# soedinglab/spacedust

Hardware: AMD Instinct MI355X
Metric: clustersearch throughput (genome-pairs/s; SW GCUPS alongside) (higher is better)
Workload: dtype int16

## Files before the change

### include/spacedust_gpu.h

```cpp
#ifndef SPACEDUST_GPU_H
#define SPACEDUST_GPU_H

#include <stddef.h>
#include <stdint.h>

#ifdef __cplusplus
extern "C" {
#endif

enum {
    SD_OK = 0,
    SD_ENODEVICE = -1,
    SD_EHIP = -2,
    SD_EINVAL = -3,
    SD_ENOMEM = -4,
    SD_EUNSUPPORTED = -5,
    SD_EMISMATCH = -6
};

typedef struct sd_ctx sd_ctx;
typedef struct sd_seqset sd_seqset;
typedef struct sd_target sd_target;

int sd_ctx_create(int device, sd_ctx **out);
int sd_ctx_create_prio(int device, int priority, sd_ctx **out);
int sd_ctx_create_masked(int device, int priority, int reserveCUs, sd_ctx **out);
void sd_ctx_destroy(sd_ctx *ctx);
const char *sd_last_error(sd_ctx *ctx);
int sd_device_name(sd_ctx *ctx, char *buf, size_t cap);
int sd_device_memory(sd_ctx *ctx, uint64_t *freeBytes, uint64_t *totalBytes);
int sd_device_identity(int device, uint64_t *id);
int sd_workspace_report(sd_ctx *ctx, uint64_t *deviceBytes, uint64_t *pinnedBytes, char *buf, size_t cap);
int sd_workspace_release(sd_ctx *ctx);
int sd_synchronize(sd_ctx *ctx);

int sd_profile_enable(sd_ctx *ctx, int on);
int sd_profile_reset(sd_ctx *ctx);
int sd_profile_get(sd_ctx *ctx, const char *name, double *totalMs, uint64_t *launches);
int sd_profile_names(sd_ctx *ctx, char *buf, size_t cap);

int sd_seqset_create(sd_ctx *ctx, const uint8_t *residues, const uint64_t *offsets, uint32_t n,
                     const int8_t *swCompBias, sd_seqset **out);
int sd_profileset_create(sd_ctx *ctx, const uint8_t *queryLetters, const uint64_t *offsets, uint32_t n,
                         const int8_t *alnProfile, sd_seqset **out);
void sd_seqset_destroy(sd_seqset *s);

typedef struct {
    int32_t gapOpen;
    int32_t gapExtend;
    int8_t matrix[21 * 21];
    int32_t covMode;
    float covThr;
    double evalThr;
    int32_t swMode;
    uint64_t dbResidues;
} sd_sw_params;

typedef struct {
    int32_t score;
    int32_t qStart, qEnd, tStart, tEnd;
    int32_t identical;
    int32_t btLen;
    int32_t flags;
    double evalue;
    uint64_t btOffset;
} sd_sw_result;

int sd_sw_align_batch(sd_ctx *ctx, const sd_sw_params *par, const sd_seqset *queries, const sd_seqset *targets,
                      uint32_t nPairs, const uint32_t *pairQ, const uint32_t *pairT, const uint8_t *isIdentity,
                      sd_sw_result *out, char *btPool, uint64_t btCap, uint64_t *btUsed);

int sd_sw_align_batch_compact(sd_ctx *ctx, const sd_sw_params *par, const sd_seqset *queries, const sd_seqset *targets,
                              uint32_t nPairs, const uint32_t *pairQ, const uint32_t *pairT, const uint8_t *isIdentity,
                              uint32_t *outIdx, sd_sw_result *out, uint32_t *nOut, char *btPool, uint64_t btCap,
                              uint64_t *btUsed);

int sd_sw_align_batch_compact_diag(sd_ctx *ctx, const sd_sw_params *par, const sd_seqset *queries, const sd_seqset *targets,
                                   uint32_t nPairs, const uint32_t *pairQ, const uint32_t *pairT, const uint16_t *pairDiag,
                                   const uint8_t *isIdentity, uint32_t *outIdx, sd_sw_result *out, uint32_t *nOut, char *btPool,
                                   uint64_t btCap, uint64_t *btUsed);

int sd_seqset_set_groups(sd_seqset *s, const uint32_t *groupOf, uint32_t nGroups, const uint32_t *keys);
int sd_sw_align_batch_best_by_group(sd_ctx *ctx, const sd_sw_params *par, const sd_seqset *queries, const sd_seqset *targets,
                                    uint32_t nPairs, const uint32_t *pairQ, const uint32_t *pairT, const uint16_t *pairDiag,
                                    const uint8_t *isIdentity, float seqIdThr, int32_t alnLenThr, uint32_t *outIdx, sd_sw_result *out,
                                    uint32_t *nOut, char *btPool, uint64_t btCap, uint64_t *btUsed);

int sd_sw_align_alt_batch(sd_ctx *ctx, const sd_sw_params *par, const sd_seqset *queries, const sd_seqset *targets, uint32_t nSeeds,
                          const uint32_t *seedQ, const uint32_t *seedT, const int32_t *tStart, const int32_t *tEnd,
                          const uint8_t *isIdentity, uint32_t maxAlt, float seqIdThr, int32_t alnLenThr, int32_t seqIdMode,
                          sd_sw_result *out, uint32_t *outCount, char *btPool, uint64_t btCap, uint64_t *btUsed);
int sd_sw_alt_last_stats(sd_ctx *ctx, uint64_t *groups, uint64_t *seedRounds, uint64_t *bytesCopied);

int sd_sw_set_cigar_pool(sd_ctx *ctx, int on);
int sd_sw_download_bytes(sd_ctx *ctx, uint64_t *recordBytes, uint64_t *poolBytes);

int sd_sw_set_narrow_final(sd_ctx *ctx, int on);

int sd_selftest_sort_pairs(sd_ctx *ctx, const uint32_t *keys, const uint32_t *vals, uint32_t n, int beginBit, int endBit, uint32_t *outKeys,
                           uint32_t *outVals);
int sd_selftest_scan(sd_ctx *ctx, const uint32_t *in, uint32_t n, uint64_t *exclusiveSum, uint32_t *runningMax);
int sd_selftest_score_class(int kernel , int32_t n, int32_t tL, int shared, int32_t wideRowLimit,
                            uint32_t *klass, char *scope, size_t cap);
int sd_selftest_r2p_weights(sd_ctx *ctx, uint32_t nTasks, const uint32_t *nRows, const uint32_t *L, const uint8_t *cells, float *freq,
                            float *eff);

int sd_sw_align_batch_hostpath(sd_ctx *ctx, const sd_sw_params *par, const sd_seqset *queries, const sd_seqset *targets,
                               uint32_t nPairs, const uint32_t *pairQ, const uint32_t *pairT, const uint8_t *isIdentity,
                               sd_sw_result *out, char *btPool, uint64_t btCap, uint64_t *btUsed);

int sd_sw_score_batch(sd_ctx *ctx, const sd_sw_params *par, const sd_seqset *queries, const sd_seqset *targets,
                      uint32_t nPairs, const uint32_t *pairQ, const uint32_t *pairT, int lanes, int reverse,
                      const int32_t *qEnd, const int32_t *tEnd, int32_t *out);

int sd_sw_last_cells(sd_ctx *ctx, uint64_t *forwardCells, uint64_t *reverseCells, uint64_t *tracebackCells);

typedef struct {
    int32_t kmerSize;
    int32_t kmerThr;
    int32_t maxHitsPerQuery;
    int32_t minDiagScore;
    uint32_t binSize;
    int32_t covMode;
    float covThr;
    int8_t ungappedMatrix[21 * 21];
} sd_prefilter_params;

typedef struct {
    uint32_t seqId;
    int32_t score;
    uint16_t diagonal;
    uint16_t pad;
} sd_hit;

int sd_target_create(sd_ctx *ctx, int kmerSize, const uint32_t *kmerOffsets, const uint32_t *entrySeq,
                     const uint16_t *entryPos, uint64_t nEntries, const uint8_t *maskedResidues,
                     const uint64_t *seqOffsets, uint32_t nSeq, const int16_t *ext2Score, const uint16_t *ext2Index,
                     const int16_t *ext3Score, const uint16_t *ext3Index, sd_target **out);
int sd_target_create_wide(sd_ctx *ctx, int kmerSize, const uint32_t *kmerOffsets, const uint64_t *kmerBlockBase,
                          const uint32_t *entrySeq, const uint16_t *entryPos, uint64_t nEntries, const uint8_t *maskedResidues,
                          const uint64_t *seqOffsets, uint32_t nSeq, const int16_t *ext2Score, const uint16_t *ext2Index,
                          const int16_t *ext3Score, const uint16_t *ext3Index, sd_target **out);
int sd_target_build(sd_ctx *ctx, int kmerSize, int kmerThr, int mask, double maskProb, const uint8_t *residues,
                    const uint64_t *seqOffsets, uint32_t nSeq, const double *maskRatios, const int8_t *selfScore,
                    const int16_t *ext2Score, const uint16_t *ext2Index, const int16_t *ext3Score, const uint16_t *ext3Index,
                    sd_target **out, uint64_t *stats);
int sd_target_sample_check(sd_ctx *ctx, const sd_target *t, const uint32_t *kmer, const uint32_t *seq, const uint32_t *pos, uint64_t n,
                           const uint32_t *sample, uint32_t nSample, uint64_t *missing, uint64_t *inSample, uint64_t resBegin,
                           uint64_t resEnd, uint8_t *maskedOut);
int sd_target_download(sd_ctx *ctx, const sd_target *t, uint64_t *nEntries, uint64_t *tableSize, uint8_t *masked, uint64_t *starts,
                       uint32_t *entrySeq, uint16_t *entryPos);
void sd_target_destroy(sd_target *t);
uint64_t sd_target_footprint(int kmerSize, uint64_t nSeq, uint64_t nResidues);
int sd_target_build_peak(const sd_target *t, uint64_t *bytes);

int sd_prefilter_batch(sd_ctx *ctx, const sd_target *target, const sd_prefilter_params *par, uint32_t nQ,
                       const uint8_t *qResidues, const uint64_t *qOffsets, const int16_t *qKmerBias,
                       const int8_t *qDiagBias, const uint32_t *identityId, sd_hit *outHits, uint32_t *outCount,
                       uint64_t *stats);

typedef struct {
    int8_t matrix[21 * 21];
    int32_t minScore;
    int32_t maxHitsPerQuery;
    int32_t covMode;
    float covThr;
} sd_ungapped_params;
int sd_ungapped_prefilter_batch(sd_ctx *ctx, const sd_ungapped_params *par, const sd_seqset *queries, const sd_seqset *targets,
                                const uint32_t *targetKeys, const uint32_t *identityId, sd_hit *outHits, uint32_t *outCount);
int sd_ungapped_score_matrix(sd_ctx *ctx, const int8_t *matrix, const sd_seqset *queries, const sd_seqset *targets, uint8_t *out);
int sd_ungapped_last_cells(sd_ctx *ctx, uint64_t *cells);

typedef struct {
    int8_t matrix[21 * 21];
    int32_t mode;
    uint8_t aa2num[256];
} sd_rescore_params;
typedef struct {
    int32_t score;
    int32_t startPos, endPos;
// ... 285 lines not shown
```

### spacedust_amd/_lib.py

```python
import ctypes as C
import os

import numpy as np

HERE = os.path.dirname(os.path.abspath(__file__))
LIB_PATH = os.path.join(HERE, 'libsdgpu.so')

_vp = C.c_void_p


SD_OK, SD_ENODEVICE, SD_EHIP, SD_EINVAL, SD_ENOMEM, SD_EUNSUPPORTED, SD_EMISMATCH = 0, -1, -2, -3, -4, -5, -6


class SdError(RuntimeError):
    pass


class SwParams(C.Structure):
    _fields_ = [('gapOpen', C.c_int32), ('gapExtend', C.c_int32), ('matrix', C.c_int8 * 441), ('covMode', C.c_int32),
                ('covThr', C.c_float), ('evalThr', C.c_double), ('swMode', C.c_int32), ('dbResidues', C.c_uint64)]


class SwResult(C.Structure):
    _fields_ = [('score', C.c_int32), ('qStart', C.c_int32), ('qEnd', C.c_int32), ('tStart', C.c_int32),
# ... 137 lines not shown
                                            _vp, C.POINTER(_vp)]),
        'sd_host_index_block_base': (C.c_int, [_vp, C.POINTER(_vp), C.POINTER(C.c_uint64)]),
        'sd_target_destroy': (None, [_vp]),
        'sd_target_build': (C.c_int, [_vp, C.c_int, C.c_int, C.c_int, C.c_double, _vp, _vp, C.c_uint32, _vp, _vp, _vp, _vp, _vp, _vp,
                                      C.POINTER(_vp), _vp]),
        'sd_target_download': (C.c_int, [_vp, _vp, C.POINTER(C.c_uint64), C.POINTER(C.c_uint64), _vp, _vp, _vp, _vp]),
        'sd_host_index_tables': (C.c_int, [_vp, _vp, _vp]),
        'sd_target_sample_check': (C.c_int, [_vp, _vp, _vp, _vp, _vp, C.c_uint64, _vp, C.c_uint32, C.POINTER(C.c_uint64), C.POINTER(C.c_uint64),
                                             C.c_uint64, C.c_uint64, _vp]),
        'sd_device_memory': (C.c_int, [_vp, C.POINTER(C.c_uint64), C.POINTER(C.c_uint64)]),
        'sd_device_identity': (C.c_int, [C.c_int, C.POINTER(C.c_uint64)]),
        'sd_workspace_report': (C.c_int, [_vp, C.POINTER(C.c_uint64), C.POINTER(C.c_uint64), C.c_char_p, C.c_size_t]),
        'sd_workspace_release': (C.c_int, [_vp]),
        'sd_prefilter_batch': (C.c_int, [_vp, _vp, C.POINTER(PrefilterParams), C.c_uint32, _vp, _vp, _vp, _vp, _vp,
                                         _vp, _vp, _vp]),
        'sd_ungapped_prefilter_batch': (C.c_int, [_vp, C.POINTER(UngappedParams), _vp, _vp, _vp, _vp, _vp, _vp]),
        'sd_ungapped_score_matrix': (C.c_int, [_vp, _vp, _vp, _vp, _vp]),
        'sd_ungapped_last_cells': (C.c_int, [_vp, C.POINTER(C.c_uint64)]),
        'sd_seqset_set_letters': (C.c_int, [_vp, _vp]),
        'sd_rescore_diagonal_batch': (C.c_int, [_vp, C.POINTER(RescoreParams), _vp, _vp, C.c_uint32, _vp, _vp, _vp, _vp]),
        'sd_search_create_ungapped': (C.c_int, [C.c_int, C.POINTER(SearchParams), C.POINTER(SetDbView), C.POINTER(_vp)]),
        'sd_comp_bias_batch': (C.c_int, [_vp, _vp, _vp, _vp, C.c_uint32, C.c_int, _vp, _vp, _vp]),
        'sd_prefilter_profile_batch': (C.c_int, [_vp, _vp, C.POINTER(PrefilterParams), C.c_uint32, _vp, _vp, _vp, _vp, _vp,
                                                 _vp, _vp, _vp, _vp]),
        'sd_profileset_create': (C.c_int, [_vp, _vp, _vp, C.c_uint32, _vp, C.POINTER(_vp)]),
        'sd_host_map_profiles': (C.c_int, [_vp, _vp, C.c_uint32, _vp, _vp, _vp, _vp, _vp, _vp]),
        'sd_host_profile_kmer_threshold': (C.c_int, [C.c_float, C.c_int]),
        'sd_clusterhits_batch': (C.c_int, [_vp, C.POINTER(ChParams), C.c_uint32, _vp, _vp, _vp, _vp, _vp, _vp, _vp,
                                           C.c_uint32, _vp, _vp, _vp, _vp, _vp, _vp]),
        'sd_agg_create': (C.c_int, [_vp, _vp, C.c_uint32, _vp, _vp, C.c_uint32, C.c_uint32, C.c_uint32, C.c_double, C.c_int,
                                    C.c_float, C.c_int, C.c_int, C.POINTER(_vp)]),
        'sd_agg_destroy': (None, [_vp]),
        'sd_agg_add': (C.c_int, [_vp, C.c_uint32, C.c_uint32, _vp, _vp, _vp, _vp, _vp]),
        'sd_agg_finish': (C.c_int, [_vp, C.POINTER(C.c_uint64), C.POINTER(C.c_uint64)]),
        'sd_agg_stats': (C.c_int, [_vp, C.POINTER(C.c_uint64), C.POINTER(C.c_uint64)]),
        'sd_agg_get': (C.c_int, [_vp, _vp, _vp, _vp, _vp, _vp, _vp]),
        'sd_agg_write_tsv': (C.c_int, [_vp, C.c_char_p, _vp, _vp, _vp, _vp, _vp, _vp, C.c_char_p, _vp, C.c_char_p, _vp,
                                       C.c_char_p, _vp, C.c_char_p, _vp, C.c_int, C.POINTER(C.c_uint64),
                                       C.POINTER(C.c_uint64)]),
        'sd_agg_write_tsv_from': (C.c_int, [_vp, C.c_char_p, C.c_int, C.c_uint64, _vp, _vp, _vp, _vp, _vp, _vp, C.c_char_p, _vp,
                                            C.c_char_p, _vp, C.c_char_p, _vp, C.c_char_p, _vp, C.c_int, C.POINTER(C.c_uint64),
                                            C.POINTER(C.c_uint64)]),
        'sd_agg_set_keys': (C.c_int, [_vp, _vp, _vp]),
        'sd_agg_set_list_order': (C.c_int, [_vp, C.c_int]),
        'sd_agg_set_pool_form': (C.c_int, [_vp, C.c_int]),
        'sd_host_matrix_text': (C.c_int, [C.c_int, C.c_char_p, C.c_size_t]),
        'sd_host_sw_comp_bias': (C.c_int, [_vp, C.c_int, _vp, _vp, C.c_uint32, _vp]),
        'sd_host_can_be_covered': (C.c_int, [C.c_float, C.c_int, C.c_float, C.c_float]),
        'sd_host_quantise_3e': (C.c_int, [C.c_double, C.c_char_p, C.POINTER(C.c_double)]),
        'sd_host_compress_backtrace': (C.c_int, [C.c_char_p, C.c_uint64, C.c_char_p, C.c_uint64, C.POINTER(C.c_uint64)]),
        'sd_host_accept_sort': (C.c_int, [C.POINTER(AlnCriteria), C.c_uint32, C.c_uint32, _vp, _vp, _vp, _vp, _vp, _vp, _vp, _vp, _vp]),
        'sd_host_realign_select': (C.c_int, [C.POINTER(AlnCriteria), C.c_uint32, _vp, _vp, _vp, _vp, _vp, _vp, _vp, _vp, _vp, _vp,
                                             _vp, _vp]),
        'sd_alntext_create': (C.c_int, [C.POINTER(_vp)]),
        'sd_alntext_destroy': (None, [_vp]),
        'sd_alntext_format': (C.c_int, [_vp, C.POINTER(AlnCriteria), C.c_uint32, _vp, _vp, _vp, _vp, _vp, _vp, _vp, _vp, _vp]),
        'sd_alntext_get': (C.c_int, [_vp, C.POINTER(C.c_char_p), C.POINTER(_vp)]),
        'sd_search_default_params': (None, [C.POINTER(SearchParams)]),
        'sd_search_create': (C.c_int, [C.c_int, C.POINTER(SearchParams), C.POINTER(SetDbView), C.POINTER(_vp)]),
        'sd_search_create_indexed': (C.c_int, [C.c_int, C.POINTER(SearchParams), C.POINTER(SetDbView), C.POINTER(IndexView), C.POINTER(_vp)]),
        'sd_search_destroy': (None, [_vp]),
        'sd_search_last_error': (C.c_char_p, [_vp]),
        'sd_search_ctx': (_vp, [_vp, C.c_int]),
        'sd_search_target': (_vp, [_vp]),
        'sd_search_set_sinks': (C.c_int, [_vp, _vp, _vp, _vp]),
        'sd_search_set_chunk_queries': (C.c_int, [_vp, C.c_int32]),
        'sd_search_set_want_records': (C.c_int, [_vp, C.c_int]),
        'sd_search_stream': (C.c_int, [_vp, C.POINTER(SetDbView), C.c_int, C.c_uint32, _vp, _vp, _vp]),
        'sd_search_result_counts': (C.c_int, [_vp, _vp]),
        'sd_search_result_arrays': (C.c_int, [_vp] + [_vp] * 12),
        'sd_search_result_write_tsv': (C.c_int, [_vp, C.c_char_p, C.c_char_p, _vp, C.c_char_p, _vp, C.c_char_p, _vp, C.c_char_p, _vp,
                                                 C.c_int, C.c_int, C.c_uint64, C.POINTER(C.c_uint64), C.POINTER(C.c_uint64)]),
        'sd_search_result_records': (C.c_int, [_vp, _vp, C.c_uint64, C.POINTER(C.c_uint64)]),
        'sd_agg_records': (C.c_int, [_vp] * 7 + [_vp, C.c_uint64, C.POINTER(C.c_uint64)]),
        'sd_records_check': (C.c_int, [_vp, C.c_uint64, C.c_uint32, C.c_uint32, C.c_uint32, C.c_uint32, C.POINTER(C.c_uint64), C.POINTER(C.c_uint64)]),
        'sd_records_write_tsv': (C.c_int, [_vp, C.c_uint64, C.c_char_p, C.c_int, C.c_uint64, C.c_char_p, _vp, C.c_char_p, _vp, C.c_char_p, _vp,
                                           C.c_char_p, _vp, C.c_int, C.POINTER(C.c_uint64), C.POINTER(C.c_uint64)]),
        'sd_search_result_destroy': (None, [_vp]),
        'sd_search_stats': (C.c_int, [_vp, _vp, _vp]),
        'sd_search_download_bytes': (C.c_int, [_vp, C.POINTER(C.c_uint64), C.POINTER(C.c_uint64)]),
        'sd_sw_set_cigar_pool': (C.c_int, [_vp, C.c_int]),
        'sd_sw_download_bytes': (C.c_int, [_vp, C.POINTER(C.c_uint64), C.POINTER(C.c_uint64)]),
        'sd_sw_set_narrow_final': (C.c_int, [_vp, C.c_int]),
        'sd_r2p_create': (C.c_int, [C.POINTER(_vp)]),
        'sd_r2p_destroy': (None, [_vp]),
        'sd_r2p_batch': (C.c_int, [_vp, C.POINTER(R2pParams), C.c_uint32] + [_vp] * 12),
        'sd_r2p_batch_device': (C.c_int, [_vp, _vp, C.POINTER(R2pParams), C.c_uint32] + [_vp] * 12),
        'sd_selftest_r2p_weights': (C.c_int, [_vp, C.c_uint32, _vp, _vp, _vp, _vp, _vp]),
        'sd_selftest_score_class': (C.c_int, [C.c_int, C.c_int32, C.c_int32, C.c_int, C.c_int32, C.POINTER(C.c_uint32), C.c_char_p, C.c_size_t]),
        'sd_shard_query_sets': (C.c_int, [_vp, C.c_uint32, C.c_uint32, C.c_uint32, _vp, C.POINTER(C.c_uint32)]),
        'sd_comm_unique_id': (C.c_int, [C.c_char_p]),
        'sd_comm_init': (C.c_int, [C.c_int, C.c_int, C.c_int, C.c_char_p, C.POINTER(_vp)]),
        'sd_comm_destroy': (None, [_vp]),
        'sd_comm_host_buffer': (C.c_int, [_vp, C.c_int, C.c_uint64, C.POINTER(_vp)]),
        'sd_comm_last_error': (C.c_char_p, [_vp]),
        'sd_search_set_records_sink': (C.c_int, [_vp, _vp, _vp]),
        'sd_gather_stream_begin': (C.c_int, [_vp, C.c_int, C.c_uint32, _vp, C.c_uint32, _vp, C.c_uint64, C.c_int, C.POINTER(_vp)]),
        'sd_gather_stream_end': (C.c_int, [_vp, _vp, _vp, C.POINTER(C.c_uint64)]),
        'sd_gather_stream_begin_tcp': (C.c_int, [_vp, C.c_int, C.c_int, C.c_uint32, _vp, C.c_uint32, _vp, C.c_uint64, C.c_int, C.POINTER(_vp)]),
        'sd_gather_results': (C.c_int, [_vp, _vp, C.c_uint64, C.c_int, _vp, _vp, C.c_uint64, C.POINTER(C.c_uint64)]),
        'sd_tcp_connect': (C.c_int, [C.c_char_p, C.c_int, C.c_int, C.c_int, C.POINTER(_vp)]),
        'sd_tcp_close': (None, [_vp]),
        'sd_tcp_bcast': (C.c_int, [_vp, _vp, C.c_uint64]),
        'sd_tcp_gather': (C.c_int, [_vp, _vp, C.c_uint64, _vp, _vp, C.c_uint64, C.POINTER(C.c_uint64)]),
    }
    missing = []
    for name, (res, args) in sig.items():
        try:
            f = getattr(L, name)
        except AttributeError:
            missing.append(name)
            continue
        f.restype = res
        f.argtypes = args
    L._sd_missing = missing
    _lib = L
    return L


def _declared_symbols():
    import re
    text = open(os.path.join(os.path.dirname(HERE), 'include', 'spacedust_gpu.h')).read()
    text = re.sub(r'/\*.*?\*/', '', text, flags=re.S)
    names = []
    for m in re.finditer(r'\b(sd_[a-z0-9_]+)\s*\(', text):
        if not re.search(r'typedef[^;]*\(\s*\*\s*%s' % m.group(1), text) and m.group(1) not in names:
            names.append(m.group(1))
    return names


DECLARED_SYMBOLS = _declared_symbols()


def ptr(a):
    return a.ctypes.data_as(C.c_void_p) if a is not None else None
```

### spacedust_amd/api.py

```python
import ctypes as C

import numpy as np

from . import _lib
from .cpus import effective_cpus
from ._lib import SdError, ptr


def _check(ctx, rc, what):
    if rc != 0:
        msg = ''
        if ctx is not None:
            msg = _lib.load().sd_last_error(ctx).decode(errors='replace')
        raise SdError('%s failed (%d): %s' % (what, rc, msg))


class Host:

    def __init__(self, threads=0):
        import os
        self.L = _lib.load()
        self.threads = threads or effective_cpus()
        h = C.c_void_p()
        _check(None, self.L.sd_host_create(self.threads, C.byref(h)), 'sd_host_create')
# ... 344 lines not shown
                                                               C.byref(used))
                else:
                    rc = self.L.sd_sw_align_batch_compact(self.h, C.byref(par), queries.h, targets.h, n, ptr(pq), ptr(pt), ptr(idt),
                                                          ptr(cidx), ptr(res), C.byref(n_out), ptr(pool), len(pool), C.byref(used))
            else:
                rc = fn(self.h, C.byref(par), queries.h, targets.h, n, ptr(pq), ptr(pt), ptr(idt), ptr(res), ptr(pool),
                        len(pool), C.byref(used))
            if rc == _lib.SD_ENOMEM and exact_cap is None:
                ql = (queries.offsets[pq + 1] - queries.offsets[pq]).astype(np.int64)
                tl = (targets.offsets[pt + 1] - targets.offsets[pt]).astype(np.int64)
                exact_cap = bt_cap = (2 if getattr(self, '_cigar_pool', False) else 1) * int((ql + tl).sum()) + 64
                continue
            _check(self.h, rc, 'sd_sw_align_batch')
            if compact:
                return cidx[:n_out.value], res[:n_out.value], pool[:used.value]
            return res, pool[:used.value]

    def sw_align_alt(self, par, queries, targets, seed_q, seed_t, t_start, t_end, max_alt, identity=None, seq_id_thr=0.0,
                     aln_len_thr=0, seq_id_mode=0, bt_cap=None):
        sq = np.ascontiguousarray(seed_q, np.uint32)
        st = np.ascontiguousarray(seed_t, np.uint32)
        tb = np.ascontiguousarray(t_start, np.int32)
        te = np.ascontiguousarray(t_end, np.int32)
        n = len(sq)
        assert len(st) == len(tb) == len(te) == n
        idt = np.ascontiguousarray(identity, np.uint8) if identity is not None else None
        ql = (queries.offsets[sq.astype(np.int64) + 1] - queries.offsets[sq]).astype(np.int64)
        tl = (targets.offsets[st.astype(np.int64) + 1] - targets.offsets[st]).astype(np.int64)
        exact = (2 if getattr(self, '_cigar_pool', False) else 1) * int(max_alt) * int((ql + tl).sum()) + 64
        if bt_cap is None:
            bt_cap = min(exact, max(1 << 20, 2 * int((ql + tl).sum()) + 64))
        res = np.zeros((n, int(max_alt)), _lib.SW_RESULT_DTYPE)
        cnt = np.zeros(n, np.uint32)
        while True:
            pool = np.zeros(bt_cap, np.uint8)
            used = C.c_uint64()
            rc = self.L.sd_sw_align_alt_batch(self.h, C.byref(par), queries.h, targets.h, n, ptr(sq), ptr(st), ptr(tb), ptr(te), ptr(idt),
                                              int(max_alt), float(seq_id_thr), int(aln_len_thr), int(seq_id_mode), ptr(res), ptr(cnt),
                                              ptr(pool), len(pool), C.byref(used))
            if rc == _lib.SD_ENOMEM and bt_cap < exact:
                bt_cap = exact
                continue
            _check(self.h, rc, 'sd_sw_align_alt_batch')
            return res, cnt, pool[:used.value]

    def sw_alt_stats(self):
        a, b, c = C.c_uint64(), C.c_uint64(), C.c_uint64()
        self.L.sd_sw_alt_last_stats(self.h, C.byref(a), C.byref(b), C.byref(c))
        return a.value, b.value, c.value

    def letterset(self, host, seqs):
        blobs = [x.encode() if isinstance(x, str) else bytes(x) for x in seqs]
        off = np.zeros(len(blobs) + 1, np.uint64)
        np.cumsum(np.fromiter((len(b) for b in blobs), np.uint64, len(blobs)), out=off[1:])
        blob = b''.join(blobs)
        res = np.zeros(len(blob), np.uint8)
        host.L.sd_host_map_sequence(host.h, blob, len(blob), ptr(res))
        s = SeqSet(self, res, off, None)
        s.set_letters(blob)
        return s

    def rescore_diagonal(self, host, queries, targets, hit_q, hit_t, hit_diag, mode=2):
        m, _, a2n = host.matrix(0)
        par = _lib.RescoreParams()
        par.mode = int(mode)
        C.memmove(par.matrix, m.ctypes.data, 441)
        C.memmove(par.aa2num, a2n.ctypes.data, 256)
        hq = np.ascontiguousarray(hit_q, np.uint32)
        ht = np.ascontiguousarray(hit_t, np.uint32)
        hd = np.ascontiguousarray(np.asarray(hit_diag, np.int64) & 0xFFFF, np.uint16)
        assert len(hq) == len(ht) == len(hd)
        out = np.zeros(len(hq), _lib.RESCORE_DTYPE)
        _check(self.h, self.L.sd_rescore_diagonal_batch(self.h, C.byref(par), queries.h, targets.h, len(hq), ptr(hq), ptr(ht), ptr(hd),
                                                        ptr(out)), 'sd_rescore_diagonal_batch')
        return out

    def set_cigar_pool(self, on=True):
        _check(self.h, self.L.sd_sw_set_cigar_pool(self.h, 1 if on else 0), 'sd_sw_set_cigar_pool')
        self._cigar_pool = bool(on)

    def set_narrow_final(self, on=True):
        _check(self.h, self.L.sd_sw_set_narrow_final(self.h, 1 if on else 0), 'sd_sw_set_narrow_final')

    def sw_download_bytes(self):
        a, b = C.c_uint64(), C.c_uint64()
        self.L.sd_sw_download_bytes(self.h, C.byref(a), C.byref(b))
        return a.value, b.value

    def sw_cells(self):
        f, r, t = C.c_uint64(), C.c_uint64(), C.c_uint64()
        self.L.sd_sw_last_cells(self.h, C.byref(f), C.byref(r), C.byref(t))
        return f.value, r.value, t.value

    def __del__(self):
        try:
            h, self.h = self.h, None
            if h:
                self.L.sd_ctx_destroy(h)
        except Exception:
            pass


class SeqSet:
    def __init__(self, ctx, residues, offsets, sw_bias, aln=None):
        self.ctx = ctx
        self.residues = np.ascontiguousarray(residues, np.uint8)
        self.offsets = np.ascontiguousarray(offsets, np.uint64)
        self.n = len(self.offsets) - 1
        b = np.ascontiguousarray(sw_bias, np.int8) if sw_bias is not None else None
        h = C.c_void_p()
        if aln is not None:
            a = np.ascontiguousarray(aln, np.int8)
            assert a.size == len(self.residues) * 21
            _check(ctx.h, ctx.L.sd_profileset_create(ctx.h, ptr(self.residues), ptr(self.offsets), self.n, ptr(a), C.byref(h)),
                   'sd_profileset_create')
        else:
            _check(ctx.h, ctx.L.sd_seqset_create(ctx.h, ptr(self.residues), ptr(self.offsets), self.n, ptr(b), C.byref(h)),
                   'sd_seqset_create')
        self.h = h

    def set_letters(self, letters):
        b = np.frombuffer(bytes(letters), np.uint8) if not isinstance(letters, np.ndarray) else np.ascontiguousarray(letters, np.uint8)
        assert len(b) == len(self.residues)
        _check(self.ctx.h, self.ctx.L.sd_seqset_set_letters(self.h, ptr(b) if len(b) else ptr(np.zeros(1, np.uint8))), 'sd_seqset_set_letters')

    def __del__(self):
        try:
            if self.ctx.h:
                self.ctx.L.sd_seqset_destroy(self.h)
        except Exception:
            pass


class Target:

    def __init__(self, ctx, host, index):
        self.ctx, self.host, self.index = ctx, host, index
        s2, i2, _ = host.ext_matrix(2)
        s3, i3, _ = host.ext_matrix(3)
        h = C.c_void_p()
        bb = getattr(index, 'block_base', None)
        _check(ctx.h, ctx.L.sd_target_create_wide(ctx.h, index.k, ptr(index.kmer_offsets), ptr(bb) if bb is not None else None,
                                                  ptr(index.entry_seq), ptr(index.entry_pos), index.n_entries, ptr(index.masked),
                                                  ptr(index.offsets), index.n, ptr(s2), ptr(i2), ptr(s3), ptr(i3),
                                                  C.byref(h)), 'sd_target_create')
        self.h = h
        self.n = index.n

    @classmethod
    def build_on_device(cls, ctx, host, residues, offsets, k=6, kmer_thr=112, mask=True, mask_prob=0.9):
        self = cls.__new__(cls)
        self.ctx, self.host, self.index = ctx, host, None
        residues = np.ascontiguousarray(residues, np.uint8)
        offsets = np.ascontiguousarray(offsets, np.uint64)
        s2, i2, _ = host.ext_matrix(2)
        s3, i3, _ = host.ext_matrix(3)
        lr = np.zeros(441, np.float64)
        self_score = np.zeros(21, np.int8)
        _check(None, host.L.sd_host_index_tables(host.h, ptr(lr), ptr(self_score)), 'sd_host_index_tables')
        h = C.c_void_p()
        stats = np.zeros(4, np.uint64)
        _check(ctx.h, ctx.L.sd_target_build(ctx.h, k, kmer_thr, 1 if mask else 0, mask_prob, ptr(residues), ptr(offsets), len(offsets) - 1,
                                            ptr(lr), ptr(self_score), ptr(s2), ptr(i2), ptr(s3), ptr(i3), C.byref(h), ptr(stats)),
               'sd_target_build')
        self.h = h
        self.n = len(offsets) - 1
# ... 165 lines not shown
```

### spacedust_amd/csrc/cli/sd_mod_iter.cpp

```cpp
#include "sd_align_core.h"
#include "sd_cli.h"
#include "sd_pref_core.h"

#include <algorithm>
#include <atomic>
#include <chrono>
#include <climits>
#include <cmath>
#include <condition_variable>
#include <cstdio>
#include <cstdlib>
#include <cstring>
#include <memory>
#include <mutex>
#include <omp.h>
#include <string>
#include <sys/resource.h>
#include <thread>
#include <vector>

namespace sdcli {

namespace {

double nowS() { return std::chrono::duration<double>(std::chrono::steady_clock::now().time_since_epoch()).count(); }
double cpuS() {
    rusage ru;
    getrusage(RUSAGE_SELF, &ru);
    return (double) ru.ru_utime.tv_sec + 1e-6 * (double) ru.ru_utime.tv_usec + (double) ru.ru_stime.tv_sec + 1e-6 * (double) ru.ru_stime.tv_usec;
}

struct Rec {
    uint32_t tId;
    uint8_t ident;
    sd_sw_result r;
};

enum { IT_PREF, IT_ALIGN, IT_R2P, IT_N };

struct ChunkOut {
    uint32_t g0 = 0, nq = 0;
    std::vector<uint32_t> pq, pt;
    std::vector<sd_sw_result> res;
    std::vector<uint8_t> ident;
    std::string pool;
    uint64_t notComputed = 0, prefHits = 0, aligned = 0, accepted = 0;
    uint64_t pfStats[5] = {0, 0, 0, 0, 0};
    int rc = SD_OK;
    std::string err;
    bool done = false;
    double sec[8][IT_N];
    double cpu[8][IT_N];
    uint64_t cnt[8][4];
};

struct Shared {
    const SeqDb *qdb = nullptr, *tdb = nullptr;
    bool sameDb = false;
    int numIt = 1, device = 0;
    sd_target *seqTarget = nullptr, *profTarget = nullptr;
    sd_seqset *tset = nullptr;
    PrefSetup pfSeq, pfProf;
    AlignSetup alFirst, alMid, alLast;
    const R2pSetup *r2p = nullptr;
    double subtractEval = 0.001;
    bool profile = false;
};

struct Worker {
    sd_ctx *ctx = nullptr;
    sd_host *host = nullptr;
    sd_r2p *r2p = nullptr;
    int threads = 1;
    QueryChunk Q;
    std::vector<uint8_t> failed;
    AlignChunk C;
    std::vector<uint32_t> mark;
    uint32_t stamp = 0;
    ~Worker() {
        if (r2p) sd_r2p_destroy(r2p);
        if (ctx) sd_sw_set_narrow_final(ctx, 0);
        if (ctx) sd_ctx_destroy(ctx);
        if (host) sd_host_destroy(host);
    }
};

double quantE(double v) {
    char text[32];
    double back = v;
    sd_host_quantise_3e(v, text, &back);
    return back;
}

int failChunk(ChunkOut &o, int rc, const std::string &what, sd_ctx *ctx) {
    o.rc = rc;
    o.err = what + " failed (" + std::to_string(rc) + ")";
    if (ctx) o.err += std::string(": ") + sd_last_error(ctx);
    return rc;
}

int processChunk(const Shared &S, Worker &W, uint32_t g0, uint32_t g1, ChunkOut &out) {
    const SeqDb &qdb = *S.qdb, &tdb = *S.tdb;
    const uint32_t nq = g1 - g0;
    out.g0 = g0;
    out.nq = nq;
    memset(out.sec, 0, sizeof(out.sec));
    memset(out.cpu, 0, sizeof(out.cpu));
    memset(out.cnt, 0, sizeof(out.cnt));
    std::vector<std::vector<Rec> > acc(nq);
    std::string &pool = out.pool;
    pool.clear();
    std::unique_ptr<SeqDb> pdb;
    QueryChunk &Q = W.Q;
    const std::vector<sd_hit> &hits = Q.hits;
    const std::vector<uint32_t> &counts = Q.counts;
    const std::vector<uint64_t> &off = Q.off;
    Q.notComputed = 0;
    W.failed.assign(nq, 0);
    if (W.mark.size() != tdb.n) W.mark.assign(tdb.n, 0);
    AlignChunk &C = W.C;
    for (int step = 0; step < S.numIt; step++) {
        const bool last = step == S.numIt - 1;
        const bool prof = step > 0;
        const SeqDb &qd = prof ? *pdb : qdb;
        const uint32_t base = prof ? 0 : g0;
        const bool sameDbStep = S.sameDb && !prof;
        const PrefSetup &PS = prof ? S.pfProf : S.pfSeq;
        double t0 = nowS(), c0 = cpuS();
        const uint64_t r0 = qd.offsets[base], r1 = qd.offsets[base + nq];
        const uint32_t Wd = (uint32_t) PS.par.maxHitsPerQuery;
        int rc = Q.run(W.ctx, W.host, prof ? S.profTarget : S.seqTarget, PS.par, PS, QuerySpan{&qd, base, &qdb, g0, nq}, tdb, sameDbStep, 0, tdb.n,
                       W.failed.data(), out.pfStats);
        if (rc != SD_OK) return failChunk(out, rc, prof ? "sd_prefilter_profile_batch" : "sd_prefilter_batch", W.ctx);
        if (Q.notComputed) {
            out.notComputed = Q.notComputed;
            out.err = Q.firstError;
        }
        out.sec[std::min(step, 7)][IT_PREF] += nowS() - t0;
        out.cpu[std::min(step, 7)][IT_PREF] += cpuS() - c0;
        t0 = nowS();
        c0 = cpuS();
        const AlignSetup &AS = step == 0 ? S.alFirst : (last ? S.alLast : S.alMid);
        C.localQ.resize(nq);
        for (uint32_t i = 0; i < nq; i++) C.localQ[i] = base + i;
        C.pq.clear();
        C.pt.clear();
        C.ident.clear();
        for (uint32_t q = 0; q < nq; q++) {
            if (prof) {
                if (++W.stamp == 0) {
                    std::fill(W.mark.begin(), W.mark.end(), 0u);
                    W.stamp = 1;
                }
                for (const Rec &e : acc[q])
                    if (quantE(e.r.evalue) <= S.subtractEval) W.mark[e.tId] = W.stamp;
            }
            const uint32_t qKey = qdb.keys[g0 + q];
            const float qL = (float) qd.lens[base + q];
            const sd_hit *row = hits.data() + (size_t) q * Wd;
            out.cnt[std::min(step, 7)][0] += counts[q];
            for (uint32_t x = 0; x < counts[q]; x++) {
                const uint32_t tId = row[x].seqId;
                if (prof && W.mark[tId] == W.stamp) continue;
                out.prefHits++;
// ... 118 lines not shown
    return SD_OK;
}

Args subArgs(const char *name, const std::vector<std::string> &flags, std::string *err) {
    std::vector<const char *> argv;
    for (const std::string &s : flags) argv.push_back(s.c_str());
    Args sub;
    sub.module = name;
    sub.parse((int) argv.size(), argv.data(), err);
    return sub;
}

}

int iterativeClusterSearchInMemory(const Args &a, const std::string &Q, const std::string &T, const std::string &tsvPath,
                                   const std::vector<std::string> &prefFlags, const std::vector<std::string> &alnFlags,
                                   const std::vector<std::string> &profFlags, const std::string &eUser, const std::string &eProfile) {
    const int numIt = (int) a.integer("--num-iterations", 1);
    const int threads = threadsOf(a);
    const int device = deviceOf(a);
    const double tStart = nowS();
    HostH host;
    if (sd_host_create(threads, &host.h) != SD_OK) return fail("sd_host_create failed");
    std::string err;
    DbPair db;
    if (!db.open(Q, T, host.h, false, true, &err)) return fail(err);
    const bool sameDb = db.sameDb;
    const SeqDb *const qdb = db.qdb, *const tdb = db.tdb.get();
    if (qdb->profile) return fail("--num-iterations starts from a sequence query DB");
    SetInfo qs, tsOwn;
    if (!qs.load(Q, true, &err)) return fail(err);
    if (!sameDb && !tsOwn.load(T, true, &err)) return fail(err);
    const SetInfo *tsP = sameDb ? &qs : &tsOwn;
    SetDbArrays tv, qv;
    tv.fill(*tdb, tsP);
    qv.fill(*qdb, &qs);
    info(a, "Query database size: %u type: Aminoacid\nTarget database size: %u type: Aminoacid\n", qdb->n, tdb->n);
    const double tLoaded = nowS();

    Shared S;
    S.qdb = qdb;
    S.tdb = tdb;
    S.sameDb = sameDb;
    S.numIt = numIt;
    S.device = device;
    S.profile = getenv("SD_ITER_PROFILE") != nullptr;
    Args prefA = subArgs("prefilter", prefFlags, &err);
    if (int rc = prefilterSetupFromArgs(prefA, host.h, *tdb, false, S.pfSeq)) return rc;
    if (int rc = prefilterSetupFromArgs(prefA, host.h, *tdb, true, S.pfProf)) return rc;
    auto alnArgs = [&](const std::string &e, bool realign) {
        std::vector<std::string> f = alnFlags;
        f.push_back("-e");
        f.push_back(e);
        f.push_back("--realign");
        f.push_back(realign ? "1" : "0");
        return subArgs("align", f, &err);
    };
    if (int rc = alignSetupFromArgs(alnArgs(eProfile, true), host.h, tdb->totalResidues(), S.alFirst)) return rc;
    if (int rc = alignSetupFromArgs(alnArgs(eProfile, false), host.h, tdb->totalResidues(), S.alMid)) return rc;
    if (int rc = alignSetupFromArgs(alnArgs(eUser, false), host.h, tdb->totalResidues(), S.alLast)) return rc;
    R2pSetup RS;
    if (int rc = r2pSetupFromArgs(subArgs("result2profile", profFlags, &err), RS)) return rc;
    S.r2p = &RS;
    {
        const double eU = strtod(eUser.c_str(), nullptr), eP = strtod(eProfile.c_str(), nullptr);
        S.subtractEval = eU < eP ? eU : eP;
    }

    int nWorkers = getenv("SD_ITER_WORKERS") ? atoi(getenv("SD_ITER_WORKERS")) : 4;
    nWorkers = std::max(1, std::min(nWorkers, 8));
    uint32_t chunkQ = (uint32_t) std::max<long long>(1, a.integer("--iter-chunk-queries", getenv("SD_ITER_CHUNK") ? atoi(getenv("SD_ITER_CHUNK")) : 1500));
    const int perWorker = std::max(1, std::min(threads, (threads * 3 / 2 + nWorkers - 1) / nWorkers));
    std::vector<std::unique_ptr<Worker> > workers;
    for (int w = 0; w < nWorkers; w++) {
        workers.emplace_back(new Worker());
        Worker &W = *workers.back();
        W.threads = perWorker;
        int rc = sd_ctx_create(device, &W.ctx);
        if (rc != SD_OK) return failNoDevice(rc);
        if (sd_host_create(perWorker, &W.host) != SD_OK) return fail("sd_host_create failed");
        if (sd_r2p_create(&W.r2p) != SD_OK) return fail("sd_r2p_create failed");
        if (S.profile) sd_profile_enable(W.ctx, 1);
        sd_sw_set_narrow_final(W.ctx, (getenv("SD_SW_NARROW_FINAL") && atoi(getenv("SD_SW_NARROW_FINAL")) == 0) ? 0 : 1);
    }
    uint64_t indexEntries = 0;
    TargetH seqTarget, profTarget;
    SeqSetH tset;
    {
        sd_ctx *c0 = workers[0]->ctx;
        uint64_t st[2] = {0, 0};
        if (int rc = buildTarget(host.h, c0, S.pfSeq, tdb->residues.data(), tdb->offsets.data(), tdb->n, &seqTarget.t, st)) return rc;
        indexEntries = st[0];
        info(a, "Index table k-mer threshold: %d at k-mer size %d\nIndex statistics\nEntries:          %llu\n", S.pfSeq.kmerThr, S.pfSeq.k,
             (unsigned long long) st[0]);
        if (numIt > 1) {
            if (int rc = buildTarget(host.h, c0, S.pfProf, tdb->residues.data(), tdb->offsets.data(), tdb->n, &profTarget.t, st, std::string(),
                                     "sd_target_build (profile searches)"))
                return rc;
            indexEntries = std::max<uint64_t>(indexEntries, st[0]);
            info(a, "Index table k-mer threshold: %d at k-mer size %d (profile iterations: every k-mer indexed)\nEntries:          %llu\n",
                 S.pfProf.kmerThr, S.pfProf.k, (unsigned long long) st[0]);
        }
        const int rc = sd_seqset_create(c0, tdb->residues.data(), tdb->offsets.data(), tdb->n, nullptr, &tset.s);
        if (rc != SD_OK) return failCtx(c0, rc, "sd_seqset_create(targets)");
    }
    S.seqTarget = seqTarget.t;
    S.profTarget = profTarget.t;
    S.tset = tset.s;
    const double tResident = nowS();
    {
        uint64_t freeB = 0, totalB = 0;
        if (sd_device_memory(workers[0]->ctx, &freeB, &totalB) == SD_OK && totalB > 0) {
            const double meanList = (double) indexEntries / 64000000.0;
            const double hitsPerSubBatch = std::min((double) (1ull << 30), (double) chunkQ * 1.3e5 * std::max(meanList, 1.0));
            const double perWorker = 26.0 * hitsPerSubBatch * 1.3 + 6e9;
            const int fit = (int) std::max(1.0, std::floor(((double) freeB - 4e9) / perWorker));
            if (fit < nWorkers) {
                info(a, "%d of %d workers: %.0f GB of device memory free, ~%.0f GB per worker\n", fit, nWorkers, (double) freeB / 1e9, perWorker / 1e9);
                nWorkers = fit;
            }
        }
    }

    struct Group {
        uint32_t b = 0, e = 0;
        size_t firstChunk = 0, nChunks = 0;
        sd_agg *agg = nullptr;
    };
    std::vector<Group> groups;
    {
        bool contiguous = true;
        for (uint32_t i = 1; i < qdb->n && contiguous; i++) contiguous = qv.setId[i] >= qv.setId[i - 1];
        if (contiguous && qdb->n) {
            uint32_t b0 = 0;
            for (uint32_t i = 1; i <= qdb->n; i++)
                if (i == qdb->n || qv.setId[i] != qv.setId[b0]) {
                    Group g;
                    g.b = b0;
                    g.e = i;
                    groups.push_back(g);
                    b0 = i;
                }
        } else if (qdb->n) {
            Group g;
            g.e = qdb->n;
            groups.push_back(g);
        }
    }
    std::vector<std::pair<uint32_t, uint32_t> > chunks;
    std::vector<size_t> groupOfChunk;
    for (size_t gi = 0; gi < groups.size(); gi++) {
        Group &g = groups[gi];
        const uint32_t n = g.e - g.b;
        const uint32_t parts = (n + chunkQ - 1) / chunkQ;
        g.firstChunk = chunks.size();
        g.nChunks = parts;
        uint32_t c0 = g.b;
        for (uint32_t x = 0; x < parts; x++) {
            const uint32_t c1 = c0 + n / parts + (x < n % parts ? 1u : 0u);
            chunks.push_back(std::make_pair(c0, c1));
            groupOfChunk.push_back(gi);
            c0 = c1;
        }
    }
    std::vector<std::unique_ptr<ChunkOut> > outs(chunks.size());
    for (auto &o : outs) o.reset(new ChunkOut());
// ... 352 lines not shown
```

### spacedust_amd/csrc/hip/sd_common.h

```cpp
#ifndef SD_COMMON_H
#define SD_COMMON_H

#include <hip/hip_runtime.h>

#include <cstdarg>
#include <cstdint>
#include <cstdio>
#include <cstring>
#include <algorithm>
#include <ctime>
#include <sys/prctl.h>
#include <map>
#include <mutex>
#include <string>
#include <vector>

#include "spacedust_gpu.h"

struct sd_profile_entry {
    double ms = 0.0;
    uint64_t launches = 0;
};

struct sd_ctx {
    int device = 0;
    hipStream_t stream = nullptr;
    std::string lastError;
    bool profiling = false;
    std::map<std::string, sd_profile_entry> profile;
    hipEvent_t evStart = nullptr, evStop = nullptr;
    bool biasTablesUploaded = false;
    hipEvent_t evSync = nullptr;
    uint64_t cellsFwd = 0, cellsRev = 0, cellsTb = 0;
    uint64_t cellsUngapped = 0;
    uint64_t altGroups = 0, altSeedRounds = 0, altBytes = 0;
    const sd_sw_result *alignDevRes = nullptr;
    size_t alignDevResN = 0;
    bool cigarPool = false;
    bool narrowFinal = false;
    uint64_t d2hRecordBytes = 0, d2hPoolBytes = 0;
    hipDeviceProp_t prop;
    struct WsEntry { void *p = nullptr; size_t bytes = 0; };
    std::map<std::string, WsEntry> ws;
    std::map<std::string, WsEntry> pinned;
    struct ProfPending { std::string name; hipEvent_t a = nullptr, b = nullptr; };
    std::vector<ProfPending> profPending;
    std::vector<hipEvent_t> evPool;
    struct PoolBuf { void *p = nullptr; size_t bytes = 0; };
    std::vector<PoolBuf> pool;
    std::mutex poolMutex;
    struct BounceBlock { uint8_t *p = nullptr; size_t cap = 0; };
    struct BounceItem { void *dst = nullptr; const uint8_t *src = nullptr; size_t bytes = 0; };
    std::vector<BounceBlock> bounce;
    std::vector<BounceItem> bounceItems;
    size_t bounceCur = 0, bounceUsed = 0;
};

inline hipError_t poolGet(sd_ctx *ctx, size_t bytes, void **out, size_t *got) {
    {
        std::lock_guard<std::mutex> lock(ctx->poolMutex);
        int best = -1;
        for (size_t i = 0; i < ctx->pool.size(); i++)
            if (ctx->pool[i].bytes >= bytes && (best < 0 || ctx->pool[i].bytes < ctx->pool[(size_t) best].bytes)) best = (int) i;
        if (best >= 0 && ctx->pool[(size_t) best].bytes <= 4 * bytes + (1u << 20)) {
            *out = ctx->pool[(size_t) best].p;
            *got = ctx->pool[(size_t) best].bytes;
            ctx->pool.erase(ctx->pool.begin() + best);
            return hipSuccess;
        }
    }
    const size_t grow = bytes + bytes / 4 + 256;
    const hipError_t e = hipMalloc(out, grow);
    *got = e == hipSuccess ? grow : 0;
    return e;
}

constexpr size_t POOL_BYTES_MAX = (size_t) 2 << 30;
inline size_t poolBytes(sd_ctx *ctx) {
    std::lock_guard<std::mutex> lock(ctx->poolMutex);
    size_t sum = 0;
    for (const sd_ctx::PoolBuf &b : ctx->pool) sum += b.bytes;
    return sum;
}
inline void poolPut(sd_ctx *ctx, void *p, size_t bytes) {
    if (!p) return;
    std::vector<void *> drop;
    {
        std::lock_guard<std::mutex> lock(ctx->poolMutex);
        if (bytes > POOL_BYTES_MAX) {
            drop.push_back(p);
        } else {
            sd_ctx::PoolBuf b;
            b.p = p;
            b.bytes = bytes;
            ctx->pool.push_back(b);
            size_t sum = 0;
            for (const sd_ctx::PoolBuf &x : ctx->pool) sum += x.bytes;
            while (ctx->pool.size() > 24 || sum > POOL_BYTES_MAX) {
                drop.push_back(ctx->pool.front().p);
                sum -= ctx->pool.front().bytes;
                ctx->pool.erase(ctx->pool.begin());
            }
        }
    }
    for (void *d : drop) (void) hipFree(d);
}

inline hipEvent_t sdProfEvent(sd_ctx *ctx) {
    if (!ctx->evPool.empty()) {
        hipEvent_t e = ctx->evPool.back();
        ctx->evPool.pop_back();
        return e;
    }
    hipEvent_t e = nullptr;
    (void) hipEventCreate(&e);
    return e;
}

inline void sdProfDrain(sd_ctx *ctx, bool wait) {
    size_t done = 0;
    for (; done < ctx->profPending.size(); done++) {
// ... 247 lines not shown
```

### spacedust_amd/csrc/hip/sd_sw.hip

```cpp
#include "sd_common.h"
#include <unistd.h>


#include <algorithm>
#include <cmath>
#include <cstring>
#include <memory>
#include <omp.h>
#include <numeric>

#include "../host/sd_host.h"
#include "sd_sw_pk.h"

namespace {

using sdpk::SwTask;
using sdpk::NARROW_EXACT;

template <int RT>
__global__ void __launch_bounds__(64)
sw_score_kernel(const SwTask *__restrict__ tasks, uint32_t nTasks, const uint8_t *__restrict__ qRes,
                const int8_t *__restrict__ qBias, const uint8_t *__restrict__ tRes, const int8_t *__restrict__ mat,
                int go, int ge, int32_t *__restrict__ out, uint2 *__restrict__ boundary,
                const uint32_t *__restrict__ order ,
// ... 605 lines not shown
    bool bad = false;
    bool going = have && reached && (i > 0 || j > 0);
    const int sh = grp * 32;
    while (__ballot(going)) {
        {
            const int ii = i - l, jj = j - l;
            bool ok = going && state == 2 && (ii > 0 || jj > 0) && ii >= 0 && jj >= 0;
            int x = ii - band;
            x = x > 0 ? x : 0;
            x = jj - x;
            ok = ok && x >= 0 && x < width_d;
            bool same = false;
            if (ok) {
                const int byte = dirs[(size_t) 16 * ii + (x >> 1)];
                const int code = (x & 1) ? (byte >> 4) : (byte & 15);
                ok = (code & 12) == 0;
                same = sq[ii] == st[jj];
            }
            const uint32_t okMask = (uint32_t) (__ballot(ok) >> sh);
            const uint32_t sameMask = (uint32_t) (__ballot(same) >> sh);
            const int run = okMask == 0xFFFFFFFFu ? 32 : __builtin_ctz(~okMask);
            const uint32_t runMask = run == 32 ? 0xFFFFFFFFu : ((1u << run) - 1u);
            if (l < run) o[-1 - l] = 'M';
            ids += __builtin_popcount(sameMask & runMask);
            i -= run;
            j -= run;
            o -= run;
            len += run;
        }
        if (going && (i > 0 || j > 0)) {
            if (i < 0 || j < 0) bad = true;
            int x = i - band;
            x = x > 0 ? x : 0;
            x = j - x;
            if (x < 0 || x >= width_d) bad = true;
            if (!bad) {
                const int byte = dirs[(size_t) 16 * i + (x >> 1)];
                const int code = (x & 1) ? (byte >> 4) : (byte & 15);
                int dcode;
                const int dE = (code & 1) ? 3 : 2, dF = (code & 2) ? 5 : 4;
                if (state == 0) dcode = dE;
                else if (state == 1) dcode = dF;
                else dcode = (code & 4) ? dE : ((code & 8) ? dF : 1);
                char c;
                switch (dcode) {
                    case 1: ids += (sq[i] == st[j]); --i; --j; state = 2; c = 'M'; break;
                    case 2: --i; state = 0; c = 'I'; break;
                    case 3: --i; state = 2; c = 'I'; break;
                    case 4: --j; state = 1; c = 'D'; break;
                    default: --j; state = 2; c = 'D'; break;
                }
                --o;
                if (l == 0) *o = c;
                len++;
            }
        }
        going = going && !bad && (i > 0 || j > 0);
    }
    if (!have || !reached || l != 0) return;
    if (bad || i != 0 || j != 0) {
        res[2 * id] = -1;
        return;
    }
    ids += (sq[0] == st[0]);
    *--o = 'M';
    len++;
    res[2 * id] = len;
    res[2 * id + 1] = ids;
}

using ScoreLaunch = void (*)(sd_ctx *ctx, const SwTask *dTasks, const uint32_t *dOrder, uint32_t n, const sd_seqset *q, const sd_seqset *t,
                             const int8_t *dMat, int go, int ge, int32_t *dOut, uint2 *dBound);

template <int RT, int LW, bool MULTI, bool WIDE, bool SHARED>
void launchScorePk(sd_ctx *ctx, const SwTask *dTasks, const uint32_t *dOrder, uint32_t n, const sd_seqset *q,
                   const sd_seqset *t, const int8_t *dMat, int go, int ge, int32_t *dOut, uint2 *dBound) {
    if (n == 0) return;
    constexpr uint32_t perWave = 2 * (64 / LW);
    dim3 grid((n + perWave - 1) / perWave), block(64);
    hipLaunchKernelGGL((sdpk::sw_score_pk_kernel<RT, LW, MULTI, WIDE, SHARED>), grid, block, 0, ctx->stream, dTasks, n, q->dRes, q->dBias,
                       t->dRes, dMat, go, ge, dOut, dBound, dOrder, (const int8_t *) q->dProf);
}

template <int RT, bool SHARED>
void launchScorePkAligned(sd_ctx *ctx, const SwTask *dTasks, const uint32_t *dOrder, uint32_t n, const sd_seqset *q, const sd_seqset *t,
                          const int8_t *dMat, int go, int ge, int32_t *dOut, uint2 * ) {
    if (n == 0) return;
    constexpr uint32_t perWave = 4;
    dim3 grid((n + perWave - 1) / perWave), block(64);
    hipLaunchKernelGGL((sdpk::sw_score_pk_aligned_kernel<RT, SHARED>), grid, block, 0, ctx->stream, dTasks, n, q->dRes, q->dBias, t->dRes,
                       dMat, go, ge, dOut, dOrder, (const int8_t *) q->dProf);
}

template <int RT>
void launchScoreIdx(sd_ctx *ctx, const SwTask *dTasks, const uint32_t *dOrder, uint32_t n, const sd_seqset *q,
                    const sd_seqset *t, const int8_t *dMat, int go, int ge, int32_t *dOut, uint2 *dBound) {
    if (n == 0) return;
    dim3 grid((n + 1) / 2), block(64);
    hipLaunchKernelGGL(sw_score_kernel<RT>, grid, block, 0, ctx->stream, dTasks, n, q->dRes, q->dBias, t->dRes, dMat,
                       go, ge, dOut, dBound, dOrder, (const int8_t *) q->dProf);
}

enum ScoreKernel { SCORE_PK = 0, SCORE_PK_WIDE = 1, SCORE_INT32 = 2 };
constexpr int SCORE_ROWS_ANY = 0x7FFFFFFF;
constexpr int I32_STRIP_ROWS = 1024;
struct ScoreSide { const char *scope; ScoreLaunch launch; };
struct ScoreClass {
    ScoreKernel form;
    int rows;
    int boundNeed;
    ScoreSide shared, unshared;
};
constexpr ScoreClass SCORE_CLASSES[] = {
    {SCORE_PK, 128, 0, {"sw_score_pk.rt4x32", launchScorePk<4, 32, false, false, true>}, {"sw_score_pk.rt4x32", launchScorePk<4, 32, false, false, false>}},
    {SCORE_PK, 160, 0, {"sw_score_pk.a_seg5", launchScorePkAligned<5, true>}, {"sw_score_pk.a_seg5", launchScorePkAligned<5, false>}},
    {SCORE_PK, 192, 0, {"sw_score_pk.a_seg6", launchScorePkAligned<6, true>}, {"sw_score_pk.a_seg6", launchScorePkAligned<6, false>}},
    {SCORE_PK, 224, 0, {"sw_score_pk.a_seg7", launchScorePkAligned<7, true>}, {"sw_score_pk.a_seg7", launchScorePkAligned<7, false>}},
    {SCORE_PK, 256, 0, {"sw_score_pk.a_seg8", launchScorePkAligned<8, true>}, {"sw_score_pk.a_seg8", launchScorePkAligned<8, false>}},
    {SCORE_PK, 288, 0, {"sw_score_pk.a_seg9", launchScorePkAligned<9, true>}, {"sw_score_pk.a_seg9", launchScorePkAligned<9, false>}},
    {SCORE_PK, 320, 0, {"sw_score_pk.a_seg10", launchScorePkAligned<10, true>}, {"sw_score_pk.a_seg10", launchScorePkAligned<10, false>}},
    {SCORE_PK, 352, 0, {"sw_score_pk.a_seg11", launchScorePkAligned<11, true>}, {"sw_score_pk.a_seg11", launchScorePkAligned<11, false>}},
    {SCORE_PK, 384, 0, {"sw_score_pk.a_seg12", launchScorePkAligned<12, true>}, {"sw_score_pk.a_seg12", launchScorePkAligned<12, false>}},
    {SCORE_PK, 416, 0, {"sw_score_pk.a_seg13", launchScorePkAligned<13, true>}, {"sw_score_pk.rt8x64", launchScorePk<8, 64, false, false, false>}},
    {SCORE_PK, 448, 0, {"sw_score_pk.a_seg14", launchScorePkAligned<14, true>}, {"sw_score_pk.rt8x64", launchScorePk<8, 64, false, false, false>}},
    {SCORE_PK, 480, 0, {"sw_score_pk.a_seg15", launchScorePkAligned<15, true>}, {"sw_score_pk.rt8x64", launchScorePk<8, 64, false, false, false>}},
    {SCORE_PK, 512, 0, {"sw_score_pk.a_seg16", launchScorePkAligned<16, true>}, {"sw_score_pk.rt8x64", launchScorePk<8, 64, false, false, false>}},
    {SCORE_PK, 544, 0, {"sw_score_pk.a_seg17", launchScorePkAligned<17, true>}, {"sw_score_pk.rt10x64", launchScorePk<10, 64, false, false, false>}},
    {SCORE_PK, 576, 0, {"sw_score_pk.a_seg18", launchScorePkAligned<18, true>}, {"sw_score_pk.rt10x64", launchScorePk<10, 64, false, false, false>}},
    {SCORE_PK, 608, 0, {"sw_score_pk.a_seg19", launchScorePkAligned<19, true>}, {"sw_score_pk.rt10x64", launchScorePk<10, 64, false, false, false>}},
    {SCORE_PK, 640, 0, {"sw_score_pk.a_seg20", launchScorePkAligned<20, true>}, {"sw_score_pk.rt10x64", launchScorePk<10, 64, false, false, false>}},
    {SCORE_PK, 672, 0, {"sw_score_pk.a_seg21", launchScorePkAligned<21, true>}, {"sw_score_pk.rt12x64", launchScorePk<12, 64, false, false, false>}},
    {SCORE_PK, 704, 0, {"sw_score_pk.a_seg22", launchScorePkAligned<22, true>}, {"sw_score_pk.rt12x64", launchScorePk<12, 64, false, false, false>}},
    {SCORE_PK, 736, 0, {"sw_score_pk.a_seg23", launchScorePkAligned<23, true>}, {"sw_score_pk.rt12x64", launchScorePk<12, 64, false, false, false>}},
    {SCORE_PK, 768, 0, {"sw_score_pk.a_seg24", launchScorePkAligned<24, true>}, {"sw_score_pk.rt12x64", launchScorePk<12, 64, false, false, false>}},
    {SCORE_PK, 1024, 2, {"sw_score_pk.rt8x64s2", launchScorePk<8, 64, true, false, true>}, {"sw_score_pk.rt8x64s2", launchScorePk<8, 64, true, false, false>}},
    {SCORE_PK, 1536, 2, {"sw_score_pk.rt8x64s3", launchScorePk<8, 64, true, false, true>}, {"sw_score_pk.rt8x64s3", launchScorePk<8, 64, true, false, false>}},
    {SCORE_PK, SCORE_ROWS_ANY, 2, {"sw_score_pk.rt8x64sN", launchScorePk<8, 64, true, false, true>}, {"sw_score_pk.rt8x64sN", launchScorePk<8, 64, true, false, false>}},
    {SCORE_PK_WIDE, 128, 0, {"sw_score_pk.w_rt4x32", launchScorePk<4, 32, false, true, true>}, {"sw_score_pk.w_rt4x32", launchScorePk<4, 32, false, true, false>}},
    {SCORE_PK_WIDE, 192, 0, {"sw_score_pk.w_rt6x32", launchScorePk<6, 32, false, true, true>}, {"sw_score_pk.w_rt6x32", launchScorePk<6, 32, false, true, false>}},
    {SCORE_PK_WIDE, 224, 0, {"sw_score_pk.w_rt7x32", launchScorePk<7, 32, false, true, true>}, {"sw_score_pk.w_rt7x32", launchScorePk<7, 32, false, true, false>}},
    {SCORE_PK_WIDE, 256, 0, {"sw_score_pk.w_rt8x32", launchScorePk<8, 32, false, true, true>}, {"sw_score_pk.w_rt8x32", launchScorePk<8, 32, false, true, false>}},
    {SCORE_PK_WIDE, 288, 0, {"sw_score_pk.w_rt9x32", launchScorePk<9, 32, false, true, true>}, {"sw_score_pk.w_rt9x32", launchScorePk<9, 32, false, true, false>}},
    {SCORE_PK_WIDE, 320, 0, {"sw_score_pk.w_rt10x32", launchScorePk<10, 32, false, true, true>}, {"sw_score_pk.w_rt10x32", launchScorePk<10, 32, false, true, false>}},
    {SCORE_PK_WIDE, 352, 0, {"sw_score_pk.w_rt11x32", launchScorePk<11, 32, false, true, true>}, {"sw_score_pk.w_rt11x32", launchScorePk<11, 32, false, true, false>}},
    {SCORE_PK_WIDE, 384, 0, {"sw_score_pk.w_rt12x32", launchScorePk<12, 32, false, true, true>}, {"sw_score_pk.w_rt12x32", launchScorePk<12, 32, false, true, false>}},
    {SCORE_PK_WIDE, 512, 0, {"sw_score_pk.w_rt8x64", launchScorePk<8, 64, false, true, true>}, {"sw_score_pk.w_rt8x64", launchScorePk<8, 64, false, true, false>}},
    {SCORE_PK_WIDE, 640, 0, {"sw_score_pk.w_rt10x64", launchScorePk<10, 64, false, true, true>}, {"sw_score_pk.w_rt10x64", launchScorePk<10, 64, false, true, false>}},
    {SCORE_PK_WIDE, 768, 0, {"sw_score_pk.w_rt12x64", launchScorePk<12, 64, false, true, true>}, {"sw_score_pk.w_rt12x64", launchScorePk<12, 64, false, true, false>}},
    {SCORE_PK_WIDE, 1024, 2, {"sw_score_pk.w_rt8x64s2", launchScorePk<8, 64, true, true, true>}, {"sw_score_pk.w_rt8x64s2", launchScorePk<8, 64, true, true, false>}},
    {SCORE_PK_WIDE, 1536, 2, {"sw_score_pk.w_rt8x64s3", launchScorePk<8, 64, true, true, true>}, {"sw_score_pk.w_rt8x64s3", launchScorePk<8, 64, true, true, false>}},
    {SCORE_PK_WIDE, SCORE_ROWS_ANY, 2, {"sw_score_pk.w_rt8x64sN", launchScorePk<8, 64, true, true, true>}, {"sw_score_pk.w_rt8x64sN", launchScorePk<8, 64, true, true, false>}},
    {SCORE_INT32, 128, 0, {"sw_score.rt4", launchScoreIdx<4>}, {"sw_score.rt4", launchScoreIdx<4>}},
    {SCORE_INT32, 256, 0, {"sw_score.rt8", launchScoreIdx<8>}, {"sw_score.rt8", launchScoreIdx<8>}},
    {SCORE_INT32, 512, 0, {"sw_score.rt16", launchScoreIdx<16>}, {"sw_score.rt16", launchScoreIdx<16>}},
    {SCORE_INT32, SCORE_ROWS_ANY, 1, {"sw_score.rt32", launchScoreIdx<32>}, {"sw_score.rt32", launchScoreIdx<32>}},
};
constexpr uint32_t N_SCORE_CLASSES = sizeof(SCORE_CLASSES) / sizeof(SCORE_CLASSES[0]);
static_assert(N_SCORE_CLASSES < 63, "class boundaries are found by one 64-lane wavefront; six class bits in the pair key");
constexpr uint32_t firstScoreClass(ScoreKernel form) {
    uint32_t ci = 0;
    while (SCORE_CLASSES[ci].form != form) ci++;
    return ci;
}
constexpr uint32_t FIRST_WIDE_CLASS = firstScoreClass(SCORE_PK_WIDE), FIRST_INT32_CLASS = firstScoreClass(SCORE_INT32);
constexpr uint32_t KEY_INVALID = N_SCORE_CLASSES * 1024u;
constexpr uint64_t scoreBoundMask(int need) {
    uint64_t m = 0;
    for (uint32_t ci = 0; ci < N_SCORE_CLASSES; ci++) m |= (uint64_t) (SCORE_CLASSES[ci].boundNeed == need) << ci;
    return m;
}
constexpr __host__ __device__ uint32_t scoreClassOf(int n, int tL, int kernel, int wideRowLimit) {
    if (kernel == SCORE_PK_WIDE && (n < tL ? n : tL) > wideRowLimit) kernel = SCORE_INT32;
    if (kernel == SCORE_INT32 || tL > 65535) return FIRST_INT32_CLASS + (n <= 128 ? 0 : (n <= 256 ? 1 : (n <= 512 ? 2 : 3)));
    const int strips = (n + 511) / 512 < 4 ? (n + 511) / 512 : 4;
    if (kernel == SCORE_PK_WIDE) {
        if (n <= 192) return FIRST_WIDE_CLASS + (n <= 128 ? 0 : 1);
        if (n <= 384) return FIRST_WIDE_CLASS + 2 + (n - 193) / 32;
        if (n <= 768) return FIRST_WIDE_CLASS + (n <= 512 ? 8 : (n <= 640 ? 9 : 10));
        return FIRST_WIDE_CLASS + 11 + strips - 2;
    }
    if (n <= 128) return 0;
    if (n <= 768) return (n + 31) / 32 - 4;
    return 21 + strips - 2;
}
constexpr bool scoreClassesAreTheTables() {
    for (int form = SCORE_PK; form <= SCORE_INT32; form++)
        for (int n = 1; n <= 2049; n++) {
            const uint32_t ci = scoreClassOf(n, 1, form, SCORE_ROWS_ANY);
            if (ci >= N_SCORE_CLASSES || SCORE_CLASSES[ci].form != form || n > SCORE_CLASSES[ci].rows) return false;
            if (ci > 0 && SCORE_CLASSES[ci - 1].form == form && n <= SCORE_CLASSES[ci - 1].rows) return false;
        }
    return true;
}
static_assert(scoreClassesAreTheTables(), "scoreClassOf: n lies in (rows of the class before, rows of its class] for every n, in every form");
static_assert(SCORE_CLASSES[N_SCORE_CLASSES - 1].form == SCORE_INT32 && SCORE_CLASSES[FIRST_INT32_CLASS - 1].form == SCORE_PK_WIDE, "forms in order");
__device__ __forceinline__ uint32_t scoreKey(int n, int tL, int kernel, int wideRowLimit = 800) {
    return scoreClassOf(n, tL, kernel, wideRowLimit) * 1024u + (uint32_t) (1023 - min(tL >> 4, 1023));
}

int runScoreTasks(sd_ctx *ctx, std::vector<SwTask> &tasks, const sd_seqset *q, const sd_seqset *t, const int8_t *dMat,
                  int go, int ge, std::vector<int32_t> &hOut, uint32_t nSlots, uint64_t *cells, const char *tag = "a") {
    hOut.assign((size_t) nSlots * 3, 0);
    if (tasks.empty()) return SD_OK;
    HostScope hsAll(ctx, "score.total");
    const size_t n = tasks.size();
    constexpr int N_I32 = N_SCORE_CLASSES - FIRST_INT32_CLASS, NB = N_I32 * 1024;
    auto keyOf = [](const SwTask &t) {
        const uint32_t ci = scoreClassOf(t.n, t.tL, SCORE_INT32, 0) - FIRST_INT32_CLASS;
        return ci * 1024u + (uint32_t) (1023 - std::min(t.tL >> 4, 1023));
    };
    SwTask *sorted = nullptr;
    SD_HIP(ctx, pinGet(ctx, (std::string("sw.tasks.") + tag).c_str(), n, &sorted));
    uint64_t boundTotal = 0, cellSum = 0;
    size_t classBegin[N_I32 + 1] = {};
    {
        int T = 1;
#pragma omp parallel
        {
#pragma omp single
            T = omp_get_num_threads();
        }
        T = std::max(1, std::min(T, 64));
        std::vector<uint32_t> hist((size_t) T * NB, 0);
#pragma omp parallel num_threads(T) reduction(+ : cellSum)
        {
            const int th = omp_get_thread_num();
            const size_t lo = n * th / T, hi = n * (th + 1) / T;
            uint32_t *hh = &hist[(size_t) th * NB];
            for (size_t i = lo; i < hi; i++) {
                hh[keyOf(tasks[i])]++;
                cellSum += (uint64_t) tasks[i].n * (uint64_t) tasks[i].tL;
            }
        }
        uint64_t run = 0;
        for (int bkt = 0; bkt < NB; bkt++) {
            if ((bkt & 1023) == 0) classBegin[bkt >> 10] = run;
            for (int th = 0; th < T; th++) {
                const uint32_t c = hist[(size_t) th * NB + bkt];
                hist[(size_t) th * NB + bkt] = (uint32_t) run;
                run += c;
            }
        }
        classBegin[N_I32] = run;
#pragma omp parallel num_threads(T)
        {
            const int th = omp_get_thread_num();
            const size_t lo = n * th / T, hi = n * (th + 1) / T;
            uint32_t *hh = &hist[(size_t) th * NB];
            for (size_t i = lo; i < hi; i++) sorted[hh[keyOf(tasks[i])]++] = tasks[i];
        }
    }
    *cells += cellSum;
    for (size_t i = classBegin[N_I32 - 1]; i < classBegin[N_I32]; i++) {
        if (sorted[i].n > I32_STRIP_ROWS) {
            sorted[i].boundOff = boundTotal;
            boundTotal += (uint64_t) sorted[i].tL;
        }
    }
    SwTask *dTasks = nullptr;
    int32_t *dOut = nullptr;
    uint2 *dBound = nullptr;
    int32_t *hPin = nullptr;
    SD_HIP(ctx, wsGet(ctx, "sw.tasks", n, &dTasks));
    SD_HIP(ctx, wsGet(ctx, "sw.out", (size_t) nSlots * 3, &dOut));
    SD_HIP(ctx, wsGet(ctx, "sw.bound", std::max<uint64_t>(boundTotal, 1), &dBound));
    SD_HIP(ctx, pinGet(ctx, "sw.hout", (size_t) nSlots * 3, &hPin));
    SD_HIP(ctx, hipMemcpyAsync(dTasks, sorted, n * sizeof(SwTask), hipMemcpyHostToDevice, ctx->stream));
    SD_HIP(ctx, hipMemsetAsync(dOut, 0, (size_t) nSlots * 3 * sizeof(int32_t), ctx->stream));
    for (int ci = 0; ci < N_I32; ci++) {
        const size_t begin = classBegin[ci], end = classBegin[ci + 1];
        if (end == begin) continue;
        {
            ProfScope ps(ctx, "sw_score");
            SCORE_CLASSES[FIRST_INT32_CLASS + ci].unshared.launch(ctx, dTasks + begin, nullptr, (uint32_t) (end - begin), q, t, dMat, go, ge, dOut, dBound);
        }
        SD_HIP(ctx, hipGetLastError());
    }
    SD_HIP(ctx, hipMemcpyAsync(hPin, dOut, (size_t) nSlots * 3 * sizeof(int32_t), hipMemcpyDeviceToHost, ctx->stream));
    SD_HIP(ctx, sdStreamSync(ctx));
    memcpy(hOut.data(), hPin, (size_t) nSlots * 3 * sizeof(int32_t));
    return SD_OK;
}


struct DevGateParams {
    int go, ge, matMin, swMode, covMode, wideRowLimit;
    float covThr;
    double evalThr;
    double lambda, K, aI, bI, alphaI, betaI, aJ, bJ, alphaJ, betaJ, sigma, tau, viThr, vjThr, cThr, dbResidues;
// ... 64 lines not shown
                best = run > best ? run : best;
            }
            pw = best >= need ? 1 : 0;
        }
    }
    preWord[i] = pw;
    pass1Keys[i] = pw ? KEY_INVALID : key;
}

__global__ void __launch_bounds__(256)
k_make_fwd(uint32_t nPairs, const uint32_t *__restrict__ pairQ, const uint32_t *__restrict__ pairT,
           const uint8_t *__restrict__ ident, const uint64_t *__restrict__ qOff, const uint64_t *__restrict__ tOff,
           SwTask *__restrict__ tasks, uint32_t *__restrict__ keys, uint32_t *__restrict__ vals,
           sd_sw_result *__restrict__ res, int usePk) {
    const uint32_t i = blockIdx.x * blockDim.x + threadIdx.x;
    if (i >= nPairs) return;
    const uint64_t qo = qOff[pairQ[i]], to = tOff[pairT[i]];
    const int qL = (int) (qOff[pairQ[i] + 1] - qo), tL = (int) (tOff[pairT[i] + 1] - to);
    SwTask tk;
    tk.qOff = qo; tk.tOff = to; tk.n = qL; tk.tL = tL; tk.qStep = 1; tk.tStep = 1;
    tk.segLen = max(1, (qL + 31) / 32);
    tk.slot = i; tk.boundOff = 0;
    const bool valid = !(ident && ident[i]) && qL > 0 && tL > 0;
    tasks[i] = tk;
    keys[i] = valid ? scoreKey(qL, tL, usePk ? SCORE_PK : SCORE_INT32) : KEY_INVALID;
    vals[i] = i;
    sd_sw_result r;
    r.score = 0; r.qStart = -1; r.qEnd = -1; r.tStart = -1; r.tEnd = -1; r.identical = 0; r.btLen = 0; r.flags = 0;
    r.evalue = 0.0; r.btOffset = 0;
    res[i] = r;
}

__global__ void k_bounds(const uint32_t *__restrict__ keys, uint32_t n, uint32_t step, uint32_t *__restrict__ b, int nb) {
    const int c = threadIdx.x;
    if (c >= nb) return;
    const uint64_t want = (uint64_t) c * step;
    uint32_t lo = 0, hi = n;
    while (lo < hi) {
        uint32_t mid = (lo + hi) >> 1;
        if ((uint64_t) keys[mid] < want) lo = mid + 1;
        else hi = mid;
    }
    b[c] = lo;
}

__global__ void __launch_bounds__(256)
k_gate_word(uint32_t nPairs, const uint32_t *__restrict__ pairQ, const int32_t *__restrict__ out32,
            const int32_t *__restrict__ minBias, int matMin, SwTask *__restrict__ tasks, uint32_t *__restrict__ keys,
            uint32_t *__restrict__ vals, uint8_t *__restrict__ word, const uint32_t *__restrict__ fwdKeys, int usePk, int wideRowLimit,
            const uint8_t *__restrict__ preWord ,
            uint8_t *__restrict__ wide ,
            unsigned long long *__restrict__ wordCount ) {
    const uint32_t i = blockIdx.x * blockDim.x + threadIdx.x;
    bool w = false, rerun = false;
    if (i < nPairs) {
        vals[i] = i;
        if (fwdKeys[i] != KEY_INVALID) {
            const int mb = minBias[pairQ[i]];
            const int bias = abs(matMin) + abs(mb);
            const bool pre = preWord && preWord[i];
            w = pre || out32[3 * i] + bias >= 255;
            rerun = w && (!wide || pre || out32[3 * i] >= NARROW_EXACT || tasks[i].tL > 65535);
        }
        word[i] = w ? 1 : 0;
        if (wide) wide[i] = rerun ? 1 : 0;
        if (w) tasks[i].segLen = max(1, (tasks[i].n + 15) / 16);
        keys[i] = rerun ? scoreKey(tasks[i].n, tasks[i].tL, usePk ? SCORE_PK_WIDE : SCORE_INT32, wideRowLimit) : KEY_INVALID;
    }
    if (wide) {
        const int nw = __popcll(__ballot(w)), nr = __popcll(__ballot(rerun));
        if ((threadIdx.x & (warpSize - 1)) == 0 && nw) {
            atomicAdd(&wordCount[0], (unsigned long long) nw);
            if (nr) atomicAdd(&wordCount[1], (unsigned long long) nr);
        }
    }
}

__global__ void __launch_bounds__(256)
k_gate_rev(uint32_t nPairs, DevGateParams gp, const uint32_t *__restrict__ pairQ, const uint32_t *__restrict__ pairT,
           const uint64_t *__restrict__ qOff, const uint64_t *__restrict__ tOff, const int32_t *__restrict__ out32,
           const int32_t *__restrict__ out16, const uint8_t *__restrict__ word, const uint32_t *__restrict__ fwdKeys,
           SwTask *__restrict__ tasks, uint32_t *__restrict__ keys, uint32_t *__restrict__ vals,
           sd_sw_result *__restrict__ res, int usePk,
           const uint8_t *__restrict__ wide ) {
    const uint32_t i = blockIdx.x * blockDim.x + threadIdx.x;
    if (i >= nPairs) return;
    vals[i] = i;
    keys[i] = KEY_INVALID;
    if (fwdKeys[i] == KEY_INVALID) return;
    const bool rerun = wide ? wide[i] != 0 : word[i] != 0;
    const int32_t *src = rerun ? &out16[3 * i] : &out32[3 * i];
    sd_sw_result r = res[i];
    r.score = src[0];
    r.tEnd = src[1];
    r.qEnd = src[2];
    r.flags = word[i] ? 1 : 0;
    if (word[i] && r.tEnd == -1) r.tEnd = 0;
    if (r.score == 0) r.qEnd = 0;
    if (r.tEnd == -1) { res[i] = r; return; }
    const uint64_t qo = qOff[pairQ[i]], to = tOff[pairT[i]];
    const int qL = (int) (qOff[pairQ[i] + 1] - qo), tL = (int) (tOff[pairT[i] + 1] - to);
    const double ev = devEvalue(gp, (double) r.score, (double) qL);
    r.evalue = ev;
    const bool lowE = ev > gp.evalThr * (1.0 + 1e-9);
    const float qCov = devCov(0, r.qEnd, qL), tCov = devCov(0, r.tEnd, tL);
    const bool lowCov = !devHasCoverage(gp.covThr, gp.covMode, qCov, tCov);
    res[i] = r;
    if (gp.swMode == 0 || lowE || lowCov) return;
    SwTask tk;
    tk.qOff = qo + r.qEnd; tk.tOff = to + r.tEnd;
    tk.n = r.qEnd + 1; tk.tL = r.tEnd + 1; tk.qStep = -1; tk.tStep = -1;
    const int lanes = word[i] ? 16 : 32;
    tk.segLen = max(1, (tk.n + lanes - 1) / lanes);
    tk.slot = i; tk.boundOff = 0;
    tasks[i] = tk;
    keys[i] = scoreKey(tk.n, tk.tL, !usePk ? SCORE_INT32 : (rerun ? SCORE_PK_WIDE : SCORE_PK), gp.wideRowLimit);
}

struct TbClass { int cap; const char *scope; };
constexpr int N_TB_NARROW = 9;
constexpr TbClass TB_CLASSES[] = {
    {128, "sw_traceback.narrow128"}, {192, "sw_traceback.narrow192"}, {256, "sw_traceback.narrow256"},
    {320, "sw_traceback.narrow320"}, {384, "sw_traceback.narrow384"}, {512, "sw_traceback.narrow512"},
    {640, "sw_traceback.narrow640"}, {768, "sw_traceback.narrow768"}, {1024, "sw_traceback.narrow1024"},
    {128, "sw_traceback.lds128"},    {512, "sw_traceback.lds512"},    {2048, "sw_traceback.lds2048"},
    {0, "sw_traceback.global"},
};
constexpr uint32_t N_TB_CLASSES = sizeof(TB_CLASSES) / sizeof(TB_CLASSES[0]), TB_GLOBAL = N_TB_CLASSES - 1;
constexpr uint32_t TBKEY_INVALID = N_TB_CLASSES * 4096u;
constexpr int TB_NARROW_ROWS = TB_CLASSES[N_TB_NARROW - 1].cap;
static_assert(TB_CLASSES[N_TB_NARROW].cap < TB_CLASSES[N_TB_NARROW - 1].cap && TB_CLASSES[TB_GLOBAL].cap == 0, "nine register-band classes first, the global class last");
__host__ __device__ __forceinline__ bool tbNarrow(int band, int qLen, int tLen) { return band * 2 + 3 <= 32 && qLen <= TB_NARROW_ROWS && tLen <= TB_NARROW_ROWS + 13; }
__host__ __device__ __forceinline__ uint32_t tbBandClass(int band) {
    uint32_t ci = N_TB_NARROW;
    while (ci < TB_GLOBAL && band * 2 + 3 > TB_CLASSES[ci].cap - 1) ci++;
    return ci;
}
__device__ __forceinline__ uint32_t tbKey(int band, int qLen, int tLen) {
    if (tbNarrow(band, qLen, tLen)) {
        uint32_t ci = 0;
        while (qLen > TB_CLASSES[ci].cap) ci++;
        const int tries = band <= 1 ? 4 : (band <= 3 ? 3 : (band <= 7 ? 2 : 1));
        return ci * 4096u + (uint32_t) (4 - tries) * 1024u + (uint32_t) (1023 - min(max(qLen - 1, 0), 1023));
    }
    const unsigned long long work = (unsigned long long) ((2 * band + 1 + 31) / 32) * (unsigned long long) qLen;
    return tbBandClass(band) * 4096u + (uint32_t) (4095 - (int) min(work >> 3, 4095ull));
}
__device__ __forceinline__ uint64_t tbDirBytes(int band, int qLen, int tLen) {
    if (tbNarrow(band, qLen, tLen)) return 0ull;
    const uint32_t ci = tbBandClass(band);
    if (ci == TB_GLOBAL)
        return (tbGlobalIntBytes(band) + (uint64_t) (band * 2 + 1) * (uint64_t) qLen + 31) & ~15ull;
    return ((uint64_t) (TB_CLASSES[ci].cap - 3) * (uint64_t) qLen + 31) & ~15ull;
}
void launchTbNarrow(sd_ctx *ctx, const sd_seqset *q, const sd_seqset *t, const int8_t *dMat, int go, int ge, const TbClass &cls, TbTask *dTb,
                    uint32_t cnt, char *dBt, int32_t *dTbRes, const uint32_t *order) {
    const int qCap = cls.cap, tCap = qCap + 16;
    const size_t ldsBytes = 2 * ((size_t) 16 * qCap + 2 * (size_t) qCap + tCap);
    auto *kernel = q->dProf ? sw_traceback_narrow_kernel<true> : sw_traceback_narrow_kernel<false>;
    hipLaunchKernelGGL(kernel, dim3((cnt + 1) / 2), dim3(64), ldsBytes, ctx->stream, dTb, cnt, q->dRes, q->dBias, t->dRes, dMat, go, ge, qCap,
                       tCap, dBt, dTbRes, order, (const int8_t *) q->dProf);
}
void launchTbBand(sd_ctx *ctx, const sd_seqset *q, const sd_seqset *t, const int8_t *dMat, int go, int ge, const TbClass &cls,
                  int maxWidthLoop, TbTask *dTb, uint32_t cnt, int8_t *dDir, char *dBt, int32_t *dTbRes, const uint32_t *order) {
    const bool global = cls.cap == 0;
    const int ldsStride = global ? INT_MAX : cls.cap + 1;
    const size_t ldsBytes = global ? 0 : (size_t) 2 * 3 * ldsStride * sizeof(int32_t);
    auto *band = global ? (q->dProf ? sw_traceback_kernel<true, true> : sw_traceback_kernel<false, true>)
                        : (q->dProf ? sw_traceback_kernel<true, false> : sw_traceback_kernel<false, false>);
    hipLaunchKernelGGL(band, dim3((cnt + 1) / 2), dim3(64), ldsBytes, ctx->stream, dTb, cnt, q->dRes, q->dBias, t->dRes, dMat, go, ge, ldsStride,
                       dDir, dBt, dTbRes, order, maxWidthLoop, (const int8_t *) q->dProf);
    auto *walk = global ? sw_traceback_walk_kernel<true> : sw_traceback_walk_kernel<false>;
    hipLaunchKernelGGL(walk, dim3((cnt + 256 / TBW_LANES - 1) / (256 / TBW_LANES)), dim3(256), 0, ctx->stream, dTb, cnt, q->dRes, t->dRes, dDir,
                       dBt, dTbRes, order);
}

__global__ void __launch_bounds__(256)
k_gate_tb(uint32_t nPairs, DevGateParams gp, const uint32_t *__restrict__ pairQ, const uint32_t *__restrict__ pairT,
          const uint64_t *__restrict__ qOff, const uint64_t *__restrict__ tOff, const int32_t *__restrict__ outRev,
          const uint32_t *__restrict__ revKeys, TbTask *__restrict__ tb, uint32_t *__restrict__ keys,
          uint32_t *__restrict__ vals, uint64_t *__restrict__ dirBytes, uint64_t *__restrict__ btBytes,
          sd_sw_result *__restrict__ res, int *__restrict__ errFlag) {
    const uint32_t i = blockIdx.x * blockDim.x + threadIdx.x;
    if (i >= nPairs) return;
    vals[i] = i;
    keys[i] = TBKEY_INVALID;
    dirBytes[i] = 0;
    btBytes[i] = 0;
    if (revKeys[i] == KEY_INVALID) return;
    sd_sw_result r = res[i];
    if (outRev[3 * i] != r.score) {
        r.flags |= 2;
        res[i] = r;
        atomicExch(errFlag, 1);
        return;
    }
    r.tStart = r.tEnd - outRev[3 * i + 1];
    r.qStart = r.qEnd - outRev[3 * i + 2];
    res[i] = r;
// ... 187 lines not shown
    if (!bbAccepted(r, B, qL, tL)) return;
    atomicMax(&table[(size_t) q * B.nGroups + B.groupOf[t]], bbPack(r, tL, B.groupKey ? B.groupKey[t] : t));
}
__global__ void __launch_bounds__(256)
k_best_keep(uint32_t nPairs, sd_sw_result *__restrict__ res, const uint8_t *__restrict__ ident, const uint32_t *__restrict__ pq,
            const uint32_t *__restrict__ pt, const uint64_t *__restrict__ qOff, const uint64_t *__restrict__ tOff, BestByGroup B,
            const unsigned long long *__restrict__ table, uint64_t *__restrict__ btLen) {
    const uint32_t i = blockIdx.x * blockDim.x + threadIdx.x;
    if (i >= nPairs || ident[i]) return;
    const uint32_t q = pq[i], t = pt[i];
    const uint32_t qL = (uint32_t) (qOff[q + 1] - qOff[q]), tL = (uint32_t) (tOff[t + 1] - tOff[t]);
    const sd_sw_result r = res[i];
    const bool keep = bbAccepted(r, B, qL, tL) &&
                      (r.evalue < B.evalExact || table[(size_t) q * B.nGroups + B.groupOf[t]] == bbPack(r, tL, B.groupKey ? B.groupKey[t] : t));
    if (!keep) {
        res[i].btLen = 0;
        btLen[i] = 0;
    }
}

__global__ void __launch_bounds__(256)
k_accept(uint32_t nPairs, const sd_sw_result *__restrict__ res, const uint8_t *__restrict__ ident, uint8_t *__restrict__ acc) {
    const uint32_t i = blockIdx.x * blockDim.x + threadIdx.x;
    if (i >= nPairs) return;
    const sd_sw_result &r = res[i];
    acc[i] = (ident[i] || (r.btLen > 0 && r.qStart >= 0 && r.tStart >= 0)) ? 1 : 0;
}
__global__ void __launch_bounds__(256)
k_accept_compact(uint32_t nPairs, const sd_sw_result *__restrict__ res, const uint8_t *__restrict__ acc,
                 const uint64_t *__restrict__ pos, sd_sw_result *__restrict__ outRes, uint32_t *__restrict__ outIdx) {
    const uint32_t i = blockIdx.x * blockDim.x + threadIdx.x;
    if (i >= nPairs || !acc[i]) return;
    outRes[pos[i]] = res[i];
    outIdx[pos[i]] = i;
}
#include "sd_scan_sort.h"

template <typename T>
int devExclusiveScan(sd_ctx *ctx, const T *in, uint64_t *out, size_t n) {
    uint64_t *tmp = nullptr;
    SD_HIP(ctx, wsGet(ctx, "al.scantmp", sdScanTmpBytes(n) / sizeof(uint64_t) + 32, &tmp));
    SD_HIP(ctx, (sdScanLaunch<T, ScanSum64, false, uint64_t>(ctx->stream, in, out, n, tmp)));
    return SD_OK;
}
int devInclusiveMax(sd_ctx *ctx, const uint32_t *in, uint32_t *out, size_t n) {
    uint32_t *tmp = nullptr;
    SD_HIP(ctx, wsGet(ctx, "al.scantmp32", sdScanTmpBytes(n) / sizeof(uint32_t) + 32, &tmp));
    SD_HIP(ctx, (sdScanLaunch<uint32_t, ScanMax32, true, uint32_t>(ctx->stream, in, out, n, tmp)));
    return SD_OK;
}

int devSortPairs(sd_ctx *ctx, const uint32_t *kIn, uint32_t *kOut, const uint32_t *vIn, uint32_t *vOut, size_t n, int endBit) {
    if (n == 0) return SD_OK;
    uint32_t *kTmp = nullptr, *vTmp = nullptr, *cnt = nullptr;
    SD_HIP(ctx, wsGet(ctx, "al.sortK", n, &kTmp));
    SD_HIP(ctx, wsGet(ctx, "al.sortV", n, &vTmp));
    SD_HIP(ctx, wsGet(ctx, "al.sortCounts", sdRadixSortCountsBytes() / sizeof(uint32_t), &cnt));
    SD_HIP(ctx, sdRadixSortPairs(ctx->stream, kIn, vIn, kOut, vOut, kTmp, vTmp, (uint32_t) n, 0, endBit, cnt));
    return SD_OK;
}

__global__ void __launch_bounds__(256)
k_bound_need(uint32_t nPairs, const SwTask *__restrict__ tasks, const uint32_t *__restrict__ keys, uint64_t *__restrict__ need) {
    const uint32_t i = blockIdx.x * blockDim.x + threadIdx.x;
    if (i >= nPairs) return;
    uint64_t v = 0;
    if (keys[i] != KEY_INVALID) {
        const uint32_t ci = keys[i] >> 10;
        constexpr uint64_t TWO = scoreBoundMask(2), ONE = scoreBoundMask(1);
        if ((TWO >> ci) & 1) v = 2ull * (uint64_t) tasks[i].tL;
        else if (((ONE >> ci) & 1) && tasks[i].n > I32_STRIP_ROWS) v = (uint64_t) tasks[i].tL;
    }
    need[i] = v;
}
__global__ void __launch_bounds__(256)
k_bound_apply(uint32_t nPairs, SwTask *__restrict__ tasks, const uint64_t *__restrict__ off) {
    const uint32_t i = blockIdx.x * blockDim.x + threadIdx.x;
    if (i >= nPairs) return;
    tasks[i].boundOff = off[i];
}

constexpr uint32_t PAIR_NONE = 0xFFFFFFFFu;
constexpr int PAIR_QUERY_BITS = 17;
__global__ void __launch_bounds__(256)
k_pair_keys(uint32_t n, const uint32_t *__restrict__ keys, const uint32_t *__restrict__ pairQ, uint32_t *__restrict__ key2) {
    const uint32_t i = blockIdx.x * blockDim.x + threadIdx.x;
    if (i >= n) return;
    const uint32_t k = keys[i];
    key2[i] = k == KEY_INVALID ? 0xFFFFFFFFu : ((k >> 10) << 26) | (pairQ[i] << 9) | ((k & 1023u) >> 1);
}
__global__ void __launch_bounds__(256)
k_pair_heads(uint32_t n, const uint32_t *__restrict__ keyS, uint32_t *__restrict__ headPos) {
    const uint32_t p = blockIdx.x * blockDim.x + threadIdx.x;
    if (p >= n) return;
    const bool head = p == 0 || (keyS[p] >> 9) != (keyS[p - 1] >> 9);
    headPos[p] = head ? p : 0u;
}
__global__ void __launch_bounds__(256)
k_pair_leaders(uint32_t n, const uint32_t *__restrict__ keyS, const uint32_t *__restrict__ runStart, uint8_t *__restrict__ leader) {
    const uint32_t p = blockIdx.x * blockDim.x + threadIdx.x;
    if (p > n) return;
    uint8_t v = 0;
    if (p < n && (keyS[p] >> 26) < FIRST_INT32_CLASS) {
        const uint32_t o = p - runStart[p];
        v = (o & 1u) == 0 ? 1 : 0;
        const bool lastOfRun = p + 1 >= n || (keyS[p + 1] >> 9) != (keyS[p] >> 9);
        const uint32_t pairs = (o + 1 + 1) / 2;
        if (lastOfRun) v += (uint8_t) (pairs & 1u);
    }
    leader[p] = v;
}
__global__ void __launch_bounds__(256)
k_pair_emit(uint32_t n, const uint32_t *__restrict__ keyS, const uint32_t *__restrict__ vals, const uint32_t *__restrict__ runStartOf,
            const uint64_t *__restrict__ pairIdx, uint32_t *__restrict__ order2) {
    const uint32_t p = blockIdx.x * blockDim.x + threadIdx.x;
    if (p >= n || (keyS[p] >> 26) >= FIRST_INT32_CLASS || ((p - runStartOf[p]) & 1u)) return;
    const uint64_t w = pairIdx[p];
    order2[2 * w] = vals[p];
    const bool mate = p + 1 < n && (keyS[p + 1] >> 9) == (keyS[p] >> 9);
    order2[2 * w + 1] = mate ? vals[p + 1] : PAIR_NONE;
}
__global__ void k_pair_bounds(const uint32_t *__restrict__ keyS, uint32_t n, const uint64_t *__restrict__ pairIdx,
                              uint32_t *__restrict__ b, int nb) {
    const int c = threadIdx.x;
    if (c >= nb) return;
    const uint32_t want = (uint32_t) c << 26;
    uint32_t lo = 0, hi = n;
    while (lo < hi) {
        const uint32_t mid = (lo + hi) >> 1;
        if (keyS[mid] < want) lo = mid + 1;
        else hi = mid;
    }
    b[c] = (uint32_t) pairIdx[lo];
}

struct AlignWs {
    size_t N;
    unsigned grid;
    int8_t *dMat;
    uint32_t *dPQ, *dPT, *dKeys, *dVals, *dKeysS, *dOrder, *dBounds, *dFwdKeys, *dRevKeys;
    uint8_t *dIdent, *dWord;
    int32_t *dMinBias, *dOut32, *dOut16, *dOutRev, *dTbRes;
    int *dErr;
    SwTask *dTasks;
    TbTask *dTb;
    sd_sw_result *dRes;
    uint64_t *dScanA, *dScanB, *dDirBytes, *dDirOff, *dBtBytes, *dBtOff, *dBtLen, *dDense;
    unsigned long long *dCells;
    char *dBt;
};

int devRunScore(sd_ctx *ctx, const AlignWs &w, uint32_t nPairs, const uint32_t *dKeys, const sd_seqset *q, const sd_seqset *t, int go, int ge,
                int32_t *dOut, const uint32_t *dPairQ ) {
    const uint32_t *dOrder = w.dOrder;
    const unsigned grid = (nPairs + 255) / 256;
    int rc = SD_OK;
    uint32_t *dOrder2 = nullptr, *dPairBounds = nullptr;
    if (dPairQ) {
        uint32_t *dKey2 = nullptr, *dVals2 = nullptr, *dHead = nullptr, *dRunStart = nullptr;
        uint64_t *dPairIdx = nullptr;
        uint8_t *dLeader = nullptr;
        SD_HIP(ctx, wsGet(ctx, "sp.key2", (size_t) nPairs, &dKey2));
        SD_HIP(ctx, wsGet(ctx, "sp.vals2", (size_t) nPairs, &dVals2));
        SD_HIP(ctx, wsGet(ctx, "sp.head", (size_t) nPairs, &dHead));
        SD_HIP(ctx, wsGet(ctx, "sp.runstart", (size_t) nPairs, &dRunStart));
        SD_HIP(ctx, wsGet(ctx, "sp.leader", (size_t) nPairs + 1, &dLeader));
        SD_HIP(ctx, wsGet(ctx, "sp.pairidx", (size_t) nPairs + 1, &dPairIdx));
        const size_t order2Cap = (size_t) 4 * nPairs + 8;
        SD_HIP(ctx, wsGet(ctx, "sp.order2", order2Cap, &dOrder2));
        SD_HIP(ctx, hipMemsetAsync(dOrder2, 0xFF, order2Cap * sizeof(uint32_t), ctx->stream));
        SD_HIP(ctx, wsGet(ctx, "sp.bounds", 64, &dPairBounds));
        hipLaunchKernelGGL(k_pair_keys, dim3(grid), dim3(256), 0, ctx->stream, nPairs, dKeys, dPairQ, dKey2);
        rc = devSortPairs(ctx, dKey2, w.dKeysS, w.dVals, dVals2, nPairs, 32);
        if (rc != SD_OK) return rc;
        dOrder = dVals2;
        hipLaunchKernelGGL(k_pair_heads, dim3(grid), dim3(256), 0, ctx->stream, nPairs, w.dKeysS, dHead);
        rc = devInclusiveMax(ctx, dHead, dRunStart, nPairs);
        if (rc != SD_OK) return rc;
        hipLaunchKernelGGL(k_pair_leaders, dim3((nPairs + 256) / 256), dim3(256), 0, ctx->stream, nPairs, w.dKeysS, dRunStart, dLeader);
        rc = devExclusiveScan(ctx, (const uint8_t *) dLeader, dPairIdx, (size_t) nPairs + 1);
        if (rc != SD_OK) return rc;
        hipLaunchKernelGGL(k_pair_emit, dim3(grid), dim3(256), 0, ctx->stream, nPairs, w.dKeysS, dVals2, dRunStart, dPairIdx, dOrder2);
        hipLaunchKernelGGL(k_pair_bounds, dim3(1), dim3(64), 0, ctx->stream, w.dKeysS, nPairs, dPairIdx, dPairBounds,
                           (int) FIRST_INT32_CLASS + 1);
        hipLaunchKernelGGL(k_bounds, dim3(1), dim3(64), 0, ctx->stream, w.dKeysS, nPairs, 1u << 26, w.dBounds, (int) N_SCORE_CLASSES + 1);
    } else {
        rc = devSortPairs(ctx, dKeys, w.dKeysS, w.dVals, w.dOrder, nPairs, 16);
        if (rc != SD_OK) return rc;
        hipLaunchKernelGGL(k_bounds, dim3(1), dim3(64), 0, ctx->stream, w.dKeysS, nPairs, 1024u, w.dBounds, (int) N_SCORE_CLASSES + 1);
    }
    hipLaunchKernelGGL(k_bound_need, dim3(grid), dim3(256), 0, ctx->stream, nPairs, w.dTasks, dKeys, w.dScanA);
    SD_HIP(ctx, hipMemsetAsync(w.dScanA + nPairs, 0, sizeof(uint64_t), ctx->stream));
    rc = devExclusiveScan(ctx, w.dScanA, w.dScanB, (size_t) nPairs + 1);
    if (rc != SD_OK) return rc;
    hipLaunchKernelGGL(k_bound_apply, dim3(grid), dim3(256), 0, ctx->stream, nPairs, w.dTasks, w.dScanB);
    uint32_t hb[N_SCORE_CLASSES + 1], hpb[FIRST_INT32_CLASS + 1];
    uint64_t boundTotal = 0;
    if (dPairQ) SD_HIP(ctx, sdD2H(ctx, hpb, dPairBounds, sizeof(hpb)));
    SD_HIP(ctx, sdD2H(ctx, hb, w.dBounds, sizeof(hb)));
    SD_HIP(ctx, sdD2H(ctx, &boundTotal, w.dScanB + nPairs, sizeof(uint64_t)));
    SD_HIP(ctx, sdStreamSync(ctx));
    uint2 *dBound = nullptr;
    SD_HIP(ctx, wsGet(ctx, "sw.bound", std::max<uint64_t>(boundTotal, 1), &dBound));
    for (uint32_t ci = 0; ci < N_SCORE_CLASSES; ci++) {
        const uint32_t begin = hb[ci], cnt = hb[ci + 1] - hb[ci];
        if (cnt == 0) continue;
        const bool shared = dPairQ != nullptr && ci < FIRST_INT32_CLASS;
        const ScoreSide &side = shared ? SCORE_CLASSES[ci].shared : SCORE_CLASSES[ci].unshared;
        ProfScope ps(ctx, side.scope);
        if (shared)
            side.launch(ctx, w.dTasks, dOrder2 + 2 * (size_t) hpb[ci], 2 * (hpb[ci + 1] - hpb[ci]), q, t, w.dMat, go, ge, dOut, dBound);
        else
            side.launch(ctx, w.dTasks, dOrder + begin, cnt, q, t, w.dMat, go, ge, dOut, dBound);
    }
    SD_HIP(ctx, hipGetLastError());
    return SD_OK;
}

__global__ void __launch_bounds__(256)
k_cells(uint32_t nPairs, const SwTask *__restrict__ tasks, const uint32_t *__restrict__ keys, unsigned long long *__restrict__ acc) {
    const uint32_t i = blockIdx.x * blockDim.x + threadIdx.x;
    unsigned long long c = 0;
    if (i < nPairs && keys[i] != KEY_INVALID) c = (unsigned long long) tasks[i].n * (unsigned long long) tasks[i].tL;
#pragma unroll
    for (int off = 32; off >= 1; off >>= 1) c += __shfl_xor(c, off, 64);
    if ((threadIdx.x & 63) == 0 && c) atomicAdd(acc, c);
}

}

int sdFail(sd_ctx *ctx, int code, const char *fmt, ...) {
    char buf[1024];
    va_list ap;
    va_start(ap, fmt);
    vsnprintf(buf, sizeof(buf), fmt, ap);
    va_end(ap);
    if (ctx) ctx->lastError = buf;
    else fprintf(stderr, "spacedust_gpu: %s\n", buf);
    return code;
}

extern "C" {

int sd_ctx_create(int device, sd_ctx **out) { return sd_ctx_create_prio(device, 0, out); }

int sd_ctx_create_prio(int device, int priority, sd_ctx **out) { return sd_ctx_create_masked(device, priority, 0, out); }

int sd_ctx_create_masked(int device, int priority, int reserveCUs, sd_ctx **out) {
    if (out == nullptr) return SD_EINVAL;
    *out = nullptr;
    int count = 0;
    hipError_t e = hipGetDeviceCount(&count);
    if (e != hipSuccess || count <= 0) {
        fprintf(stderr, "spacedust_gpu: no HIP device visible (%s); this library has no CPU fallback\n",
                e != hipSuccess ? hipGetErrorString(e) : "device count 0");
        return SD_ENODEVICE;
    }
    if (device < 0 || device >= count) return SD_EINVAL;
    if (hipSetDevice(device) != hipSuccess) return SD_ENODEVICE;
    sd_ctx *c = new sd_ctx();
    c->device = device;
    int least = 0, greatest = 0;
    (void) hipDeviceGetStreamPriorityRange(&least, &greatest);
    const int prio = priority < 0 ? greatest : (priority > 0 ? least : (least + greatest) / 2);
    hipError_t se = hipSuccess;
    (void) hipGetDeviceProperties(&c->prop, device);
    const int nCU = c->prop.multiProcessorCount;
    if (reserveCUs > 0 && nCU > 0 && reserveCUs < nCU) {
        std::vector<uint32_t> mask((size_t) (nCU + 31) / 32, 0u);
        for (int b = 0; b < nCU - reserveCUs; b++) mask[(size_t) b / 32] |= 1u << (b % 32);
        se = hipExtStreamCreateWithCUMask(&c->stream, (uint32_t) mask.size(), mask.data());
    } else {
        se = hipStreamCreateWithPriority(&c->stream, hipStreamNonBlocking, prio);
    }
    if (se != hipSuccess) {
        delete c;
        return SD_EHIP;
    }
    const char *syncMode = getenv("SD_SYNC");
    const bool spin = syncMode && strcmp(syncMode, "spin") == 0;
    (void) hipEventCreate(&c->evStart);
    (void) hipEventCreate(&c->evStop);
    if (!spin) (void) hipEventCreateWithFlags(&c->evSync, hipEventDisableTiming);
    (void) hipGetDeviceProperties(&c->prop, device);
    *out = c;
    return SD_OK;
}

void sd_ctx_destroy(sd_ctx *ctx) {
    if (!ctx) return;
// ... 662 lines not shown
            } else if (btPool) {
                memset(btPool + btPos, 'M', L);
                r.btOffset = btPos;
                btPos += L;
            }
        }
    }
    if (a.btUsed) *a.btUsed = btPos;
    ctx->d2hRecordBytes += (uint64_t) nRec * (sizeof(sd_sw_result) + (a.compactIdx ? sizeof(uint32_t) : 0));
    ctx->d2hPoolBytes += poolBytes;
    return SD_OK;
}

static int alignBatchImpl(sd_ctx *ctx, const AlignCall &a) {
    const sd_sw_params *par = a.par;
    const sd_seqset *queries = a.queries, *targets = a.targets;
    const uint32_t nPairs = a.nPairs;
    if (!ctx || !par || !queries || !targets || !a.out) return SD_EINVAL;
    if (a.compactIdx && (!a.nCompact || par->swMode != 2)) return sdFail(ctx, SD_EINVAL, "the compact variants need swMode 2 (records with backtraces)");
    (void) hipSetDevice(ctx->device);
    sdD2HReset(ctx);
    if (a.btUsed) *a.btUsed = 0;
    if (a.nCompact) *a.nCompact = 0;
    if (nPairs == 0) return SD_OK;
    const int go = par->gapOpen, ge = par->gapExtend;
    ctx->cellsFwd = ctx->cellsRev = ctx->cellsTb = 0;
    sd::Evaluer ev;
    sd::initEvaluer(ev, par->dbResidues);
    int matMin = 0;
    for (int i = 0; i < 441; i++) matMin = std::min(matMin, (int) par->matrix[i]);
    for (uint32_t i = 0; i < nPairs; i++)
        if (a.pairQ[i] >= queries->n || a.pairT[i] >= targets->n) return sdFail(ctx, SD_EINVAL, "pair %u out of range", i);
    if (targets->dProf) return sdFail(ctx, SD_EUNSUPPORTED, "profile targets are not implemented (profile queries are)");
    std::unique_ptr<HostScope> hs(new HostScope(ctx, "align.upload"));
    DevGateParams gp;
    gp.go = go; gp.ge = ge; gp.matMin = matMin; gp.swMode = par->swMode; gp.covMode = par->covMode; gp.covThr = par->covThr;
    {
        int matMax = 0;
        for (int x = 0; x < 441; x++) matMax = std::max(matMax, (int) par->matrix[x]);
        const int maxEntry = std::max(1, queries->dProf ? queries->maxEntryAdd : matMax + queries->maxEntryAdd);
        gp.wideRowLimit = 32767 / maxEntry;
    }
    gp.evalThr = par->evalThr;
    gp.lambda = ev.lambda; gp.K = ev.K; gp.aI = ev.aI; gp.bI = ev.bI; gp.alphaI = ev.alphaI; gp.betaI = ev.betaI;
    gp.aJ = ev.aJ; gp.bJ = ev.bJ; gp.alphaJ = ev.alphaJ; gp.betaJ = ev.betaJ; gp.sigma = ev.sigma; gp.tau = ev.tau;
    gp.viThr = ev.viThr; gp.vjThr = ev.vjThr; gp.cThr = ev.cThr; gp.dbResidues = ev.dbResidues;
    AlignWs w = {};
    int rc = alignWsInit(ctx, a, w);
    if (rc != SD_OK) return rc;
    const size_t N = w.N;
    const unsigned grid = w.grid;

    hs.reset(new HostScope(ctx, "align.fwd32"));
    const int usePk = (go >= ge && go < 1024 && ge >= 0 && getenv("SD_SW_INT32") == nullptr) ? 1 : 0;
    hipLaunchKernelGGL(k_make_fwd, dim3(grid), dim3(256), 0, ctx->stream, nPairs, w.dPQ, w.dPT, w.dIdent, queries->dOff, targets->dOff,
                       w.dTasks, w.dFwdKeys, w.dVals, w.dRes, usePk);
    uint32_t *dPass1Keys = w.dFwdKeys;
    uint8_t *dPreWord = nullptr, *dWide = nullptr;
    const bool narrowFinal = ctx->narrowFinal && usePk;
    if (narrowFinal) SD_HIP(ctx, wsGet(ctx, "al.wide", N, &dWide));
    if (a.pairDiag && usePk) {
        uint16_t *dDiag = nullptr;
        SD_HIP(ctx, wsGet(ctx, "al.diag", N, &dDiag));
        SD_HIP(ctx, wsGet(ctx, "al.preword", N, &dPreWord));
        SD_HIP(ctx, wsGet(ctx, "al.pass1keys", N, &dPass1Keys));
        SD_HIP(ctx, hipMemcpyAsync(dDiag, a.pairDiag, N * sizeof(uint16_t), hipMemcpyHostToDevice, ctx->stream));
        hipLaunchKernelGGL(k_pre_word, dim3(grid), dim3(256), 0, ctx->stream, nPairs, (const uint32_t *) w.dPQ, (const uint32_t *) w.dPT,
                           (const uint16_t *) dDiag, (const uint32_t *) w.dFwdKeys, (const uint64_t *) queries->dOff, (const uint64_t *) targets->dOff,
                           (const uint8_t *) queries->dRes, (const int8_t *) queries->dBias, (const uint8_t *) targets->dRes, (const int8_t *) w.dMat,
                           (const int8_t *) queries->dProf, (const int32_t *) w.dMinBias, queries->dProf ? 0 : matMin, dPreWord, dPass1Keys,
                           narrowFinal ? 1 : 0);
    }
    hipLaunchKernelGGL(k_cells, dim3(grid), dim3(256), 0, ctx->stream, nPairs, w.dTasks, dPass1Keys, w.dCells + 0);
    const uint32_t *dShare = queries->n >= (1u << PAIR_QUERY_BITS) ? nullptr : w.dPQ;
    rc = devRunScore(ctx, w, nPairs, dPass1Keys, queries, targets, go, ge, w.dOut32, dShare);
    if (rc != SD_OK) return rc;
    hs.reset(new HostScope(ctx, "align.fwd16"));
    hipLaunchKernelGGL(k_gate_word, dim3(grid), dim3(256), 0, ctx->stream, nPairs, w.dPQ, w.dOut32, w.dMinBias, queries->dProf ? 0 : matMin, w.dTasks, w.dKeys,
                       w.dVals, w.dWord, w.dFwdKeys, usePk, gp.wideRowLimit, (const uint8_t *) dPreWord, dWide, w.dCells + 2);
    hipLaunchKernelGGL(k_cells, dim3(grid), dim3(256), 0, ctx->stream, nPairs, w.dTasks, w.dKeys, w.dCells + 0);
    rc = devRunScore(ctx, w, nPairs, w.dKeys, queries, targets, go, ge, w.dOut16, dShare);
    if (rc != SD_OK) return rc;
    hs.reset(new HostScope(ctx, "align.rev"));
    hipLaunchKernelGGL(k_gate_rev, dim3(grid), dim3(256), 0, ctx->stream, nPairs, gp, w.dPQ, w.dPT, queries->dOff, targets->dOff, w.dOut32,
                       w.dOut16, w.dWord, w.dFwdKeys, w.dTasks, w.dRevKeys, w.dVals, w.dRes, usePk, (const uint8_t *) dWide);
    hipLaunchKernelGGL(k_cells, dim3(grid), dim3(256), 0, ctx->stream, nPairs, w.dTasks, w.dRevKeys, w.dCells + 1);
    rc = devRunScore(ctx, w, nPairs, w.dRevKeys, queries, targets, go, ge, w.dOutRev, nullptr);
    if (rc != SD_OK) return rc;
    hs.reset(new HostScope(ctx, "align.traceback"));
    hipLaunchKernelGGL(k_gate_tb, dim3(grid), dim3(256), 0, ctx->stream, nPairs, gp, w.dPQ, w.dPT, queries->dOff, targets->dOff, w.dOutRev,
                       w.dRevKeys, w.dTb, w.dKeys, w.dVals, w.dDirBytes, w.dBtBytes, w.dRes, w.dErr);
    SD_HIP(ctx, hipMemsetAsync(w.dBtBytes + N, 0, sizeof(uint64_t), ctx->stream));
    rc = devExclusiveScan(ctx, w.dBtBytes, w.dBtOff, N + 1);
    if (rc != SD_OK) return rc;
    uint64_t btScratch = 0;
    SD_HIP(ctx, sdD2H(ctx, &btScratch, w.dBtOff + N, sizeof(uint64_t)));
    SD_HIP(ctx, sdStreamSync(ctx));
    SD_HIP(ctx, wsGet(ctx, "tb.bt", btScratch + 64, &w.dBt));
    rc = runTracebackRounds(ctx, a, w);
    if (rc != SD_OK) return rc;
    if (getenv("SD_DEBUG_TB")) {
        rc = printTracebackStats(ctx, w, nPairs);
        if (rc != SD_OK) return rc;
    }
    if (a.bestBy && a.compactIdx && targets->dGroupOf && targets->nGroups > 0 && (uint64_t) queries->n * targets->nGroups <= (1ull << 27)) {
        rc = markBestByGroup(ctx, a, w);
        if (rc != SD_OK) return rc;
    }
    hs.reset(new HostScope(ctx, "align.download"));
    AlignRecords rec;
    rc = downloadRecords(ctx, a, w, narrowFinal, rec);
    if (rc != SD_OK) return rc;
    hs.reset(new HostScope(ctx, "align.finish"));
    return finishRecordsOnHost(ctx, a, ev, rec);
}

int sd_sw_set_cigar_pool(sd_ctx *ctx, int on) {
    if (!ctx) return SD_EINVAL;
    ctx->cigarPool = on != 0;
    return SD_OK;
}

int sd_sw_set_narrow_final(sd_ctx *ctx, int on) {
    if (!ctx) return SD_EINVAL;
    ctx->narrowFinal = on != 0;
    return SD_OK;
}

int sd_sw_download_bytes(sd_ctx *ctx, uint64_t *recordBytes, uint64_t *poolBytes) {
    if (!ctx) return SD_EINVAL;
    if (recordBytes) *recordBytes = ctx->d2hRecordBytes;
    if (poolBytes) *poolBytes = ctx->d2hPoolBytes;
    return SD_OK;
}

int sd_sw_align_batch(sd_ctx *ctx, const sd_sw_params *par, const sd_seqset *queries, const sd_seqset *targets,
                      uint32_t nPairs, const uint32_t *pairQ, const uint32_t *pairT, const uint8_t *isIdentity,
                      sd_sw_result *out, char *btPool, uint64_t btCap, uint64_t *btUsed) {
    return alignBatchImpl(ctx, {par, queries, targets, nPairs, pairQ, pairT, isIdentity, out, btPool, btCap, btUsed, nullptr, nullptr, nullptr, nullptr});
}

int sd_sw_align_batch_compact(sd_ctx *ctx, const sd_sw_params *par, const sd_seqset *queries, const sd_seqset *targets,
                              uint32_t nPairs, const uint32_t *pairQ, const uint32_t *pairT, const uint8_t *isIdentity,
                              uint32_t *outIdx, sd_sw_result *out, uint32_t *nOut, char *btPool, uint64_t btCap,
                              uint64_t *btUsed) {
    if (!outIdx || !nOut) return SD_EINVAL;
    return alignBatchImpl(ctx, {par, queries, targets, nPairs, pairQ, pairT, isIdentity, out, btPool, btCap, btUsed, outIdx, nOut, nullptr, nullptr});
}

int sd_sw_align_batch_compact_diag(sd_ctx *ctx, const sd_sw_params *par, const sd_seqset *queries, const sd_seqset *targets,
                                   uint32_t nPairs, const uint32_t *pairQ, const uint32_t *pairT, const uint16_t *pairDiag,
                                   const uint8_t *isIdentity, uint32_t *outIdx, sd_sw_result *out, uint32_t *nOut, char *btPool,
                                   uint64_t btCap, uint64_t *btUsed) {
    if (!outIdx || !nOut) return SD_EINVAL;
    return alignBatchImpl(ctx, {par, queries, targets, nPairs, pairQ, pairT, isIdentity, out, btPool, btCap, btUsed, outIdx, nOut, pairDiag, nullptr});
}

int sd_selftest_sort_pairs(sd_ctx *ctx, const uint32_t *keys, const uint32_t *vals, uint32_t n, int beginBit, int endBit, uint32_t *outKeys,
                           uint32_t *outVals) {
    if (!ctx || (n && (!keys || !vals || !outKeys || !outVals)) || beginBit < 0 || endBit > 32 || beginBit >= endBit) return SD_EINVAL;
    if (n == 0) return SD_OK;
    (void) hipSetDevice(ctx->device);
    DevBuf<uint32_t> kIn, vIn, kOut, vOut, kTmp, vTmp, cnt;
    SD_HIP(ctx, kIn.alloc(n));
    SD_HIP(ctx, vIn.alloc(n));
    SD_HIP(ctx, kOut.alloc(n));
    SD_HIP(ctx, vOut.alloc(n));
    SD_HIP(ctx, kTmp.alloc(n));
    SD_HIP(ctx, vTmp.alloc(n));
    SD_HIP(ctx, cnt.alloc(sdRadixSortCountsBytes() / sizeof(uint32_t)));
    SD_HIP(ctx, hipMemcpy(kIn.p, keys, (size_t) n * 4, hipMemcpyHostToDevice));
    SD_HIP(ctx, hipMemcpy(vIn.p, vals, (size_t) n * 4, hipMemcpyHostToDevice));
    SD_HIP(ctx, sdRadixSortPairs(ctx->stream, kIn.p, vIn.p, kOut.p, vOut.p, kTmp.p, vTmp.p, n, beginBit, endBit, cnt.p));
    SD_HIP(ctx, hipStreamSynchronize(ctx->stream));
    SD_HIP(ctx, hipMemcpy(outKeys, kOut.p, (size_t) n * 4, hipMemcpyDeviceToHost));
    SD_HIP(ctx, hipMemcpy(outVals, vOut.p, (size_t) n * 4, hipMemcpyDeviceToHost));
    return SD_OK;
}

int sd_selftest_scan(sd_ctx *ctx, const uint32_t *in, uint32_t n, uint64_t *exclusiveSum, uint32_t *runningMax) {
    if (!ctx || !in || !exclusiveSum || n == 0) return SD_EINVAL;
    (void) hipSetDevice(ctx->device);
    DevBuf<uint32_t> dIn, dMax;
    DevBuf<uint64_t> dOut;
    SD_HIP(ctx, dIn.alloc((size_t) n + 1));
    SD_HIP(ctx, dOut.alloc((size_t) n + 1));
    SD_HIP(ctx, hipMemset(dIn.p, 0, ((size_t) n + 1) * 4));
    SD_HIP(ctx, hipMemcpy(dIn.p, in, (size_t) n * 4, hipMemcpyHostToDevice));
    int rc = devExclusiveScan(ctx, (const uint32_t *) dIn.p, dOut.p, (size_t) n + 1);
    if (rc != SD_OK) return rc;
    if (runningMax) {
        SD_HIP(ctx, dMax.alloc(n));
        rc = devInclusiveMax(ctx, dIn.p, dMax.p, n);
        if (rc != SD_OK) return rc;
    }
    SD_HIP(ctx, hipStreamSynchronize(ctx->stream));
    SD_HIP(ctx, hipMemcpy(exclusiveSum, dOut.p, ((size_t) n + 1) * 8, hipMemcpyDeviceToHost));
    if (runningMax) SD_HIP(ctx, hipMemcpy(runningMax, dMax.p, (size_t) n * 4, hipMemcpyDeviceToHost));
    return SD_OK;
}

int sd_selftest_score_class(int kernel, int32_t n, int32_t tL, int shared, int32_t wideRowLimit, uint32_t *klass, char *scope, size_t cap) {
    if (kernel < SCORE_PK || kernel > SCORE_INT32 || n < 1 || tL < 1 || !klass || (cap && !scope)) return SD_EINVAL;
    const uint32_t ci = scoreClassOf(n, tL, kernel, wideRowLimit);
    const ScoreSide &side = shared && ci < FIRST_INT32_CLASS ? SCORE_CLASSES[ci].shared : SCORE_CLASSES[ci].unshared;
    *klass = ci;
    if (cap) snprintf(scope, cap, "%s", side.scope);
    return SD_OK;
}

int sd_sw_align_batch_best_by_group(sd_ctx *ctx, const sd_sw_params *par, const sd_seqset *queries, const sd_seqset *targets,
                                    uint32_t nPairs, const uint32_t *pairQ, const uint32_t *pairT, const uint16_t *pairDiag,
                                    const uint8_t *isIdentity, float seqIdThr, int32_t alnLenThr, uint32_t *outIdx, sd_sw_result *out,
                                    uint32_t *nOut, char *btPool, uint64_t btCap, uint64_t *btUsed) {
    if (!outIdx || !nOut || !targets) return SD_EINVAL;
    if (!targets->dGroupOf) return sdFail(ctx, SD_EINVAL, "sd_sw_align_batch_best_by_group: the target set has no groups (sd_seqset_set_groups)");
    const float bb[2] = {seqIdThr, (float) alnLenThr};
    return alignBatchImpl(ctx, {par, queries, targets, nPairs, pairQ, pairT, isIdentity, out, btPool, btCap, btUsed, outIdx, nOut, pairDiag, bb});
}

int sd_sw_align_batch_hostpath(sd_ctx *ctx, const sd_sw_params *par, const sd_seqset *queries, const sd_seqset *targets,
                      uint32_t nPairs, const uint32_t *pairQ, const uint32_t *pairT, const uint8_t *isIdentity,
                      sd_sw_result *out, char *btPool, uint64_t btCap, uint64_t *btUsed) {
    if (!ctx || !par || !queries || !targets || !out) return SD_EINVAL;
    if (queries->dProf || targets->dProf) return sdFail(ctx, SD_EUNSUPPORTED, "the host-orchestrated A/B path takes sequence sets only");
    (void) hipSetDevice(ctx->device);
    const int go = par->gapOpen, ge = par->gapExtend;
    ctx->cellsFwd = ctx->cellsRev = ctx->cellsTb = 0;
    sd::Evaluer ev;
    sd::initEvaluer(ev, par->dbResidues);
    int matMin = 0;
    for (int i = 0; i < 441; i++) matMin = std::min(matMin, (int) par->matrix[i]);
    DevBuf<int8_t> dMat;
    SD_HIP(ctx, dMat.alloc(441));
    SD_HIP(ctx, hipMemcpy(dMat.p, par->matrix, 441, hipMemcpyHostToDevice));
    if (btUsed) *btUsed = 0;
    uint64_t btPos = 0;

    std::unique_ptr<HostScope> hs(new HostScope(ctx, "align.init"));
    std::vector<int> qLv(nPairs), tLv(nPairs);
    for (uint32_t i = 0; i < nPairs; i++) {
        if (pairQ[i] >= queries->n || pairT[i] >= targets->n) return sdFail(ctx, SD_EINVAL, "pair %u out of range", i);
        qLv[i] = (int) (queries->hOff[pairQ[i] + 1] - queries->hOff[pairQ[i]]);
        tLv[i] = (int) (targets->hOff[pairT[i] + 1] - targets->hOff[pairT[i]]);
        sd_sw_result &r = out[i];
        r.score = 0; r.qStart = -1; r.qEnd = -1; r.tStart = -1; r.tEnd = -1; r.identical = 0; r.btLen = 0; r.flags = 0;
        r.evalue = 0.0; r.btOffset = 0;
    }
    for (uint32_t i = 0; i < nPairs; i++) {
        if (!(isIdentity && isIdentity[i])) continue;
        sd_sw_result &r = out[i];
        const int rcI = scoreIdentical(ctx, par, ev, queries, targets, i, pairQ[i], pairT[i], r);
        if (rcI != SD_OK) return rcI;
        if (btPool) {
            if (btPos + (uint64_t) r.btLen > btCap) return sdFail(ctx, SD_ENOMEM, "backtrace pool too small");
            memset(btPool + btPos, 'M', r.btLen);
            r.btOffset = btPos;
            btPos += r.btLen;
        }
    }
    hs.reset(new HostScope(ctx, "align.fwd32"));
    std::vector<SwTask> tasks;
    {
        std::vector<uint32_t> keepIdx(nPairs);
        uint32_t nKeep = 0;
        for (uint32_t i = 0; i < nPairs; i++)
            if (!(isIdentity && isIdentity[i]) && qLv[i] > 0 && tLv[i] > 0) keepIdx[nKeep++] = i;
        tasks.resize(nKeep);
#pragma omp parallel for schedule(static)
        for (uint32_t x = 0; x < nKeep; x++) tasks[x] = fwdTask(queries, targets, pairQ[keepIdx[x]], pairT[keepIdx[x]], keepIdx[x], 32);
    }
    std::vector<int32_t> h;
    int rc = runScoreTasks(ctx, tasks, queries, targets, dMat.p, go, ge, h, nPairs, &ctx->cellsFwd, "f32");
    if (rc != SD_OK) return rc;
    hs.reset(new HostScope(ctx, "align.fwd16"));
    std::vector<SwTask> tasks2;
    std::vector<uint8_t> word(nPairs, 0);
    for (size_t x = 0; x < tasks.size(); x++) {
        const uint32_t i = tasks[x].slot;
        const int bias = std::abs(matMin) + std::abs(queries->hMinBias[pairQ[i]]);
        if (h[3 * i] + bias >= 255) {
            word[i] = 1;
            tasks2.push_back(fwdTask(queries, targets, pairQ[i], pairT[i], i, 16));
        }
    }
    std::vector<int32_t> h2;
    rc = runScoreTasks(ctx, tasks2, queries, targets, dMat.p, go, ge, h2, nPairs, &ctx->cellsFwd, "f16");
    if (rc != SD_OK) return rc;
// ... 160 lines not shown
```

### spacedust_amd/csrc/hip/sd_sw_pk.h

```cpp
#ifndef SD_SW_PK_H
#define SD_SW_PK_H

#include <hip/hip_runtime.h>
#include <cstdint>

namespace sdpk {

struct SwTask {
    uint64_t qOff;
    uint64_t tOff;
    int32_t n;
    int32_t tL;
    int32_t qStep;
    int32_t tStep;
    int32_t segLen;
    uint32_t slot;
    uint64_t boundOff;
};

typedef short s16x2 __attribute__((ext_vector_type(2)));
typedef unsigned short u16x2 __attribute__((ext_vector_type(2)));

__device__ __forceinline__ uint32_t pkMax(uint32_t a, uint32_t b) {
    return __builtin_bit_cast(uint32_t, __builtin_elementwise_max(__builtin_bit_cast(s16x2, a), __builtin_bit_cast(s16x2, b)));
// ... 255 lines not shown
                        const unsigned long long lo = (unsigned long long) outG | ((unsigned long long) outFf << 32);
                        __hip_atomic_store((unsigned long long *) &bnd[c], lo, __ATOMIC_RELAXED, __HIP_MEMORY_SCOPE_AGENT);
                    }
                }
                if (WIDE) {
                    const bool upA = cmA > (bestA | 0xFFFFu), upB = cmB > (bestB | 0xFFFFu);
                    bestA = upA ? cmA : bestA;
                    bcolA = upA ? ccol : bcolA;
                    bestB = upB ? cmB : bestB;
                    bcolB = upB ? ccol : bcolB;
                } else {
                    const uint32_t v = pkLshr(cm, 5);
                    const uint32_t nb = pkMax(bestv, v);
                    const uint32_t m = pkAshr(pkSub(bestv, nb), 15);
                    bestcm = bfi(m, cm, bestcm);
                    bestcol = bfi(m, ccol, bestcol);
                    bestv = nb;
                }
                ccol = pkAdd(ccol, 0x00010001u);
            }
            chunk = chunkNext;
            bchunk = bnext;
        }
        {
            const uint32_t vA = WIDE ? bestA >> 16 : bestv & 0xFFFFu, vB = WIDE ? bestB >> 16 : bestv >> 16;
            const uint32_t rcA = WIDE ? bestA & 31u : bestcm & 31u, rcB = WIDE ? bestB & 31u : (bestcm >> 16) & 31u;
            const uint32_t rowA = (uint32_t) (q0 + 31 - (int) rcA), rowB = (uint32_t) (q0 + 31 - (int) rcB);
            const uint32_t colA = WIDE ? bcolA & 0xFFFFu : bestcol & 0xFFFFu, colB = WIDE ? bcolB >> 16 : bestcol >> 16;
            if (vA > 0) {
                const unsigned long long kk = ((unsigned long long) vA << 40) | ((unsigned long long) (0xFFFFFu - colA) << 20) |
                                              (unsigned long long) (0xFFFFFu - rowA);
                keyA = kk > keyA ? kk : keyA;
            }
            if (vB > 0) {
                const unsigned long long kk = ((unsigned long long) vB << 40) | ((unsigned long long) (0xFFFFFu - colB) << 20) |
                                              (unsigned long long) (0xFFFFFu - rowB);
                keyB = kk > keyB ? kk : keyB;
            }
        }
    }
#pragma unroll
    for (int off = LW / 2; off >= 1; off >>= 1) {
        const unsigned long long oa = __shfl_xor(keyA, off, LW), ob = __shfl_xor(keyB, off, LW);
        keyA = oa > keyA ? oa : keyA;
        keyB = ob > keyB ? ob : keyB;
    }
    if (l == 0) {
        if (haveA) {
            const int v = (int) (keyA >> 40);
            out[3 * A.slot + 0] = v;
            out[3 * A.slot + 1] = v == 0 ? -1 : 0xFFFFF - (int) ((keyA >> 20) & 0xFFFFF);
            out[3 * A.slot + 2] = v == 0 ? A.n - 1 : 0xFFFFF - (int) (keyA & 0xFFFFF);
        }
        if (haveB) {
            const int v = (int) (keyB >> 40);
            out[3 * B.slot + 0] = v;
            out[3 * B.slot + 1] = v == 0 ? -1 : 0xFFFFF - (int) ((keyB >> 20) & 0xFFFFF);
            out[3 * B.slot + 2] = v == 0 ? B.n - 1 : 0xFFFFF - (int) (keyB & 0xFFFFF);
        }
    }
}

__device__ __forceinline__ uint32_t pkAshr15(uint32_t a) {
    uint32_t r;
    asm("v_pk_ashrrev_i16 %0, 15, %1 op_sel_hi:[0,1]" : "=v"(r) : "v"(a));
    return r;
}
__device__ __forceinline__ uint32_t bfiAsm(uint32_t mask, uint32_t a, uint32_t b) {
    uint32_t r;
    asm("v_bfi_b32 %0, %1, %2, %3" : "=v"(r) : "v"(mask), "v"(a), "v"(b));
    return r;
}
__device__ __forceinline__ uint32_t addWord0(uint32_t base, uint32_t packed) {
    uint32_t r;
    asm("v_add_u32_sdwa %0, %1, %2 dst_sel:DWORD dst_unused:UNUSED_PAD src0_sel:DWORD src1_sel:WORD_0" : "=v"(r) : "v"(base), "v"(packed));
    return r;
}
__device__ __forceinline__ uint32_t addWord1(uint32_t base, uint32_t packed) {
    uint32_t r;
    asm("v_add_u32_sdwa %0, %1, %2 dst_sel:DWORD dst_unused:UNUSED_PAD src0_sel:DWORD src1_sel:WORD_1" : "=v"(r) : "v"(base), "v"(packed));
    return r;
}

template <int RT, bool SHARED>
__global__ void __launch_bounds__(64)
sw_score_pk_aligned_kernel(const SwTask *__restrict__ tasks, uint32_t nTasks, const uint8_t *__restrict__ qRes,
                           const int8_t *__restrict__ qBias, const uint8_t *__restrict__ tRes, const int8_t *__restrict__ mat,
                           int go, int ge, int32_t *__restrict__ out, const uint32_t *__restrict__ order,
                           const int8_t *__restrict__ qProf) {
    constexpr int LW = 32;
    constexpr int WORDS = (RT + 3) / 4;
    constexpr int RTP = 4 * WORDS;
    constexpr int PSTRIDE = LW * WORDS;
    constexpr int NGRP = 64 / LW;
    constexpr int NT = 2 * NGRP;
    constexpr uint32_t ROWB = PSTRIDE * 4;
    static_assert(22 * ROWB < 65536, "row offsets travel in 16 bits");
    __shared__ uint32_t prof[SHARED ? 1 : NT][22][PSTRIDE];
    __shared__ int8_t smat[441];
    for (int i = threadIdx.x; i < 441; i += 64) smat[i] = mat[i];
    __syncthreads();
    const int lane = threadIdx.x & 63, wave = threadIdx.x >> 6;
    const int grp = lane / LW, l = lane % LW;
    SwTask tk[NT];
#pragma unroll
    for (int x = 0; x < NT; x++) {
        const uint32_t id = (blockIdx.x + (uint32_t) wave) * NT + x;
        const uint32_t tid = id < nTasks ? (order ? order[id] : id) : 0xFFFFFFFFu;
        if (tid != 0xFFFFFFFFu) {
            tk[x] = tasks[tid];
        } else {
            tk[x].n = 0; tk[x].tL = 0; tk[x].qOff = 0; tk[x].tOff = 0; tk[x].qStep = 1; tk[x].tStep = 1; tk[x].segLen = 1;
            tk[x].slot = 0; tk[x].boundOff = 0;
        }
    }
    SwTask A = tk[0], B = tk[1];
#pragma unroll
    for (int g = 1; g < NGRP; g++)
        if (grp == g) {
            A = tk[2 * g];
            B = tk[2 * g + 1];
        }
    const bool haveA = A.n > 0, haveB = B.n > 0;
    if (SHARED && !haveB) {
        B = A;
        B.tL = 0;
    }
    int maxN = 0, maxTL = 0;
#pragma unroll
    for (int x = 0; x < NT; x++) {
        maxN = max(maxN, tk[x].n);
        maxTL = max(maxTL, tk[x].tL);
    }
    const int steps = (maxN > 0 && maxTL > 0) ? maxTL + LW - 1 : 0;
    const uint32_t goP = (uint32_t) go | ((uint32_t) go << 16), geP = (uint32_t) ge | ((uint32_t) ge << 16);
    const int q0 = l * RT;
#pragma unroll
    for (int x = 0; x < (SHARED ? 1 : 2); x++) {
        const SwTask &T = SHARED ? tk[0] : (x ? B : A);
        uint32_t *pw = &prof[SHARED ? 0 : 2 * grp + x][0][0] + l * WORDS;
#pragma unroll
        for (int w = 0; w < WORDS; w++) {
            int res[4], cb[4];
            int64_t pidx[4];
            bool valid[4];
#pragma unroll
            for (int b = 0; b < 4; b++) {
                const int qi = q0 + 4 * w + b;
                valid[b] = (4 * w + b < RT) && qi < T.n;
                res[b] = 20;
                cb[b] = 0;
                pidx[b] = 0;
                if (valid[b]) {
                    const int64_t idx = (int64_t) T.qOff + (int64_t) qi * T.qStep;
                    res[b] = qRes[idx];
                    cb[b] = qBias[idx];
                    pidx[b] = idx * 21;
                }
            }
            const int aFirst = SHARED ? wave * NGRP + grp : 0, aStep = SHARED ? NGRP : 1;
            if (qProf) {
                for (int a = aFirst; a < 21; a += aStep) {
                    uint32_t word = 0;
#pragma unroll
                    for (int b = 0; b < 4; b++) {
                        const int v = valid[b] ? (int) qProf[pidx[b] + a] : -64;
                        word |= (uint32_t) (uint8_t) (int8_t) v << (8 * b);
                    }
                    pw[a * PSTRIDE + w] = word;
                }
            } else {
                for (int a = aFirst; a < 21; a += aStep) {
                    uint32_t word = 0;
#pragma unroll
                    for (int b = 0; b < 4; b++) {
                        const int v = valid[b] ? (int) smat[a * 21 + res[b]] + cb[b] : -64;
                        word |= (uint32_t) (uint8_t) (int8_t) v << (8 * b);
                    }
                    pw[a * PSTRIDE + w] = word;
                }
            }
            pw[PK_NEUTRAL * PSTRIDE + w] = 0xC0C0C0C0u;
        }
    }
    __syncthreads();
    typedef __attribute__((address_space(3))) uint32_t lds_u32;
    const uint32_t baseA = (uint32_t) (size_t) (lds_u32 *) (&prof[SHARED ? 0 : 2 * grp][0][0] + l * WORDS);
    const uint32_t baseB = SHARED ? baseA : (uint32_t) (size_t) (lds_u32 *) (&prof[2 * grp + 1][0][0] + l * WORDS);
    auto ldsWord = [](uint32_t addr, int w) -> uint32_t { return *((const lds_u32 *) (size_t) addr + w); };

    uint32_t H[RTP], E[RTP];
#pragma unroll
    for (int r = 0; r < RTP; r++) {
        H[r] = 0;
        E[r] = 0;
    }
    uint32_t outG = 0, outFf = 0, prevInG = 0;
    uint32_t bestcm = 0, bestcol = 0;
    constexpr uint32_t NEUT = (uint32_t) PK_NEUTRAL * ROWB;
    auto loadChunk = [&](int c0) -> uint32_t {
        const int col = c0 + l;
        uint32_t a = PK_NEUTRAL, b = PK_NEUTRAL;
        if (col < A.tL) a = tRes[(int64_t) A.tOff + (int64_t) col * A.tStep];
        if (col < B.tL) b = tRes[(int64_t) B.tOff + (int64_t) col * B.tStep];
        return (a * ROWB) | ((b * ROWB) << 16);
    };
    uint32_t chunk = loadChunk(0);
    uint32_t chunkNext = loadChunk(LW);
    uint32_t T = NEUT | (NEUT << 16);
    T = writeLane<0>(readLane(chunk, 0), T);
    T = writeLane<32>(readLane(chunk, 32), T);
    uint32_t pa[WORDS], pb[WORDS];
    {
        const uint32_t aA = addWord0(baseA, T), aB = addWord1(baseB, T);
#pragma unroll
        for (int w = 0; w < WORDS; w++) {
            pa[w] = ldsWord(aA, w);
            pb[w] = ldsWord(aB, w);
        }
    }
    auto columnStep = [&](const int k, const uint32_t &Tc, const uint32_t (&pac)[WORDS], const uint32_t (&pbc)[WORDS], uint32_t &Tn,
                          uint32_t (&pan)[WORDS], uint32_t (&pbn)[WORDS]) {
        const int i1 = (k + 1) & (LW - 1);
        if (i1 == 0) {
            chunk = chunkNext;
            chunkNext = loadChunk(k + 1 + LW);
        }
        Tn = dppShr1(Tc);
        Tn = writeLane<0>(readLane(chunk, i1), Tn);
        Tn = writeLane<32>(readLane(chunk, 32 + i1), Tn);
        {
            const uint32_t aA = addWord0(baseA, Tn), aB = addWord1(baseB, Tn);
#pragma unroll
            for (int w = 0; w < WORDS; w++) {
                pan[w] = ldsWord(aA, w);
                pbn[w] = ldsWord(aB, w);
            }
        }
        uint32_t inG = dppShr1(outG), inFf = dppShr1(outFf);
        inG = writeLane<32>(0, inG);
        inFf = writeLane<32>(0, inFf);
        uint32_t h[RTP];
#pragma unroll
        for (int w = 0; w < WORDS; w++) {
            const uint32_t d0 = (w == 0) ? prevInG : H[4 * w - 1];
            addProfile4(pac[w], pbc[w], d0, H[4 * w], H[4 * w + 1], H[4 * w + 2], h[4 * w], h[4 * w + 1], h[4 * w + 2], h[4 * w + 3]);
        }
        prevInG = inG;
        uint32_t Ff = inFf, cm = 0;
#pragma unroll
        for (int r = 0; r < RT; r++) {
            const uint32_t hpre = pkMax(h[r], E[r]);
            const uint32_t g = pkMax(hpre, Ff);
            const uint32_t open = pkSubSat(hpre, goP);
            E[r] = pkMax(pkSubSat(E[r], geP), open);
            Ff = pkMax(pkSubSat(Ff, geP), open);
            H[r] = g;
            const uint32_t code = pkRowCode(g, 31 - r);
            cm = r == 0 ? code : pkMax(cm, code);
        }
        outG = H[RT - 1];
        outFf = Ff;
        const uint32_t t = bestcm | 0x001F001Fu;
        const uint32_t m = pkAshr15(pkSub(t, cm));
        const uint32_t kk = (uint32_t) k | ((uint32_t) k << 16);
        bestcm = bfiAsm(m, cm, bestcm);
        bestcol = bfiAsm(m, kk, bestcol);
    };
    uint32_t T2, pa2[WORDS], pb2[WORDS];
#pragma unroll 1
    for (int k = 0; k < steps; k += 2) {
        columnStep(k, T, pa, pb, T2, pa2, pb2);
        columnStep(k + 1, T2, pa2, pb2, T, pa, pb);
    }
    unsigned long long keyA = 0, keyB = 0;
    {
        const uint32_t vA = (bestcm & 0xFFFFu) >> 5, vB = bestcm >> 21;
        const uint32_t rowA = (uint32_t) (q0 + 31 - (int) (bestcm & 31u)), rowB = (uint32_t) (q0 + 31 - (int) ((bestcm >> 16) & 31u));
        const uint32_t colA = (bestcol & 0xFFFFu) - (uint32_t) l, colB = (bestcol >> 16) - (uint32_t) l;
        if (vA > 0) keyA = ((unsigned long long) vA << 40) | ((unsigned long long) (0xFFFFFu - colA) << 20) | (unsigned long long) (0xFFFFFu - rowA);
        if (vB > 0) keyB = ((unsigned long long) vB << 40) | ((unsigned long long) (0xFFFFFu - colB) << 20) | (unsigned long long) (0xFFFFFu - rowB);
    }
#pragma unroll
    for (int off = LW / 2; off >= 1; off >>= 1) {
        const unsigned long long oa = __shfl_xor(keyA, off, LW), ob = __shfl_xor(keyB, off, LW);
        keyA = oa > keyA ? oa : keyA;
        keyB = ob > keyB ? ob : keyB;
    }
    if (l == 0) {
        if (haveA) {
            const int v = (int) (keyA >> 40);
            out[3 * A.slot + 0] = v;
            out[3 * A.slot + 1] = v == 0 ? -1 : 0xFFFFF - (int) ((keyA >> 20) & 0xFFFFF);
            out[3 * A.slot + 2] = v == 0 ? A.n - 1 : 0xFFFFF - (int) (keyA & 0xFFFFF);
        }
        if (haveB) {
            const int v = (int) (keyB >> 40);
            out[3 * B.slot + 0] = v;
            out[3 * B.slot + 1] = v == 0 ? -1 : 0xFFFFF - (int) ((keyB >> 20) & 0xFFFFF);
            out[3 * B.slot + 2] = v == 0 ? B.n - 1 : 0xFFFFF - (int) (keyB & 0xFFFFF);
        }
    }
}

}
#endif
```

### spacedust_amd/csrc/host/sd_search.cpp

```cpp
#include "sd_host.h"
#include "sd_target_build.h"
#include "spacedust_gpu.h"

#include <algorithm>
#include <chrono>
#include <condition_variable>
#include <cstdio>
#include <cstdlib>
#include <cstring>
#include <deque>
#include <fstream>
#include <functional>
#include <future>
#include <memory>
#include <mutex>
#include <string>
#include <thread>
#include <pthread.h>
#include <vector>

namespace {

double nowSec() {
    return std::chrono::duration<double>(std::chrono::steady_clock::now().time_since_epoch()).count();
// ... 380 lines not shown
}

int sd_search_set_chunk_queries(sd_search *s, int32_t chunkQueries) {
    if (!s || chunkQueries < 0) return SD_EINVAL;
    s->par.chunkQueries = chunkQueries;
    return SD_OK;
}

int sd_search_set_records_sink(sd_search *s, sd_records_sink fn, void *user) {
    if (!s) return SD_EINVAL;
    s->recordsSink = fn;
    s->recordsSinkUser = user;
    return SD_OK;
}

int sd_search_set_want_records(sd_search *s, int on) {
    if (!s) return SD_EINVAL;
    s->wantRecords = on != 0;
    return SD_OK;
}

int sd_search_stats(sd_search *s, uint64_t *stats, double *seconds) {
    if (!s) return SD_EINVAL;
    if (stats) memcpy(stats, s->stats, sizeof(s->stats));
    if (seconds) memcpy(seconds, s->seconds, sizeof(s->seconds));
    return SD_OK;
}

int sd_search_download_bytes(sd_search *s, uint64_t *recordBytes, uint64_t *poolBytes) {
    if (!s) return SD_EINVAL;
    uint64_t rec = 0, pool = 0;
    sd_ctx *al[4] = {s->ctxAl, s->ctxAl2, s->ctxAlMore[0], s->ctxAlMore[1]};
    for (sd_ctx *c : al) {
        uint64_t a = 0, b = 0;
        if (c && sd_sw_download_bytes(c, &a, &b) == SD_OK) {
            rec += a;
            pool += b;
        }
    }
    if (recordBytes) *recordBytes = rec;
    if (poolBytes) *poolBytes = pool;
    return SD_OK;
}

int sd_search_stream(sd_search *s, const sd_setdb *Q, int sameDb, uint32_t nRanges, const uint32_t *rangeBegin,
                     const uint32_t *rangeEnd, sd_search_result **results) {
    if (!s || !Q || !results || (nRanges && (!rangeBegin || !rangeEnd))) return SD_EINVAL;
    const bool profile = Q->alnProfile != nullptr;
    if (profile != (s->par.profileQueries != 0)) return s->fail(SD_EINVAL, "sd_search_stream: query DB type does not match profileQueries");
    if (profile && (!Q->sortedScore || !Q->sortedIndex)) return SD_EINVAL;
    const double tAll = nowSec();
    const sd_setdb &T = s->T;
    std::vector<int32_t> qLen(Q->n);
    for (uint32_t i = 0; i < Q->n; i++) qLen[i] = (int32_t) (Q->offsets[i + 1] - Q->offsets[i]);
    const bool aggregate = Q->setId && Q->posInSet && Q->strand && T.setId && T.posInSet && T.strand;
    const bool pushdown = aggregate && !s->alnSink && !(getenv("SD_EVAL_PUSHDOWN") && atoi(getenv("SD_EVAL_PUSHDOWN")) == 0);
    s->swParRun = s->swPar;
    if (pushdown) s->swParRun.evalThr = std::min(s->swPar.evalThr, 1.2e-6);
    s->stats[S_EVAL_PUSHDOWN] = pushdown ? 1 : 0;
    s->bestOnDevice = pushdown && s->targetHasGroups && !(getenv("SD_BEST_ON_DEVICE") && atoi(getenv("SD_BEST_ON_DEVICE")) == 0);
    s->cigarOnDevice = aggregate && !s->alnSink && !(getenv("SD_CIGAR_ON_DEVICE") && atoi(getenv("SD_CIGAR_ON_DEVICE")) == 0);
    struct CigarMode {
        sd_ctx *al[4];
        explicit CigarMode(sd_search *s_, bool on) : al{s_->ctxAl, s_->ctxAl2, s_->ctxAlMore[0], s_->ctxAlMore[1]} {
            for (sd_ctx *c : al)
                if (c) sd_sw_set_cigar_pool(c, on ? 1 : 0);
        }
        ~CigarMode() {
            for (sd_ctx *c : al)
                if (c) sd_sw_set_cigar_pool(c, 0);
        }
    } cigarMode(s, s->cigarOnDevice);
    struct NarrowFinalMode {
        sd_ctx *al[4];
        explicit NarrowFinalMode(sd_search *s_, bool on) : al{s_->ctxAl, s_->ctxAl2, s_->ctxAlMore[0], s_->ctxAlMore[1]} {
            for (sd_ctx *c : al)
                if (c) sd_sw_set_narrow_final(c, on ? 1 : 0);
        }
        ~NarrowFinalMode() {
            for (sd_ctx *c : al)
                if (c) sd_sw_set_narrow_final(c, 0);
        }
    } narrowFinalMode(s, !(getenv("SD_SW_NARROW_FINAL") && atoi(getenv("SD_SW_NARROW_FINAL")) == 0));
    std::vector<uint32_t> qSetSize(Q->nSets, 0);
    if (aggregate)
        for (uint32_t i = 0; i < Q->n; i++)
            if (Q->setId[i] < Q->nSets) qSetSize[Q->setId[i]]++;
    if (aggregate) {
        uint32_t m = 0;
        for (uint32_t v : qSetSize) m = std::max(m, v);
        for (uint32_t v : s->tSetSize) m = std::max(m, v);
        for (uint32_t i = 0; i < Q->n; i++) m = std::max(m, Q->posInSet[i]);
        for (uint32_t i = 0; i < T.n; i++) m = std::max(m, T.posInSet[i]);
        if (s->lgamma.size() < (size_t) m + 8) {
            s->lgamma.resize((size_t) m + 8);
            sd_host_lgamma_table(s->lgamma.data(), (uint32_t) s->lgamma.size());
        }
    }
    std::vector<std::unique_ptr<sd_search_result> > res(nRanges);
    for (uint32_t r = 0; r < nRanges; r++) {
        res[r].reset(new sd_search_result());
        if (!aggregate) continue;
        int rc = sd_agg_create(Q->setId, qLen.data(), Q->n, T.setId, s->tLen.data(), T.n, Q->nSets, T.nSets, s->par.evalThr, s->par.covMode,
                               s->par.covThr, s->par.alnLenThr, s->par.filterSelfMatch, &res[r]->agg);
        if (rc != SD_OK) return s->fail(rc, "sd_agg_create");
        if (Q->keys || T.keys) sd_agg_set_keys(res[r]->agg, Q->keys, T.keys);
        if (s->cigarOnDevice) sd_agg_set_pool_form(res[r]->agg, 1);
    }
    struct Chunk {
        uint32_t range, c0, c1;
    };
    std::vector<Chunk> chunks;
    const uint32_t chunkQ = (uint32_t) (s->par.chunkQueries > 0 ? s->par.chunkQueries : (T.n >= 1000000u ? 2500 : 10000));
    for (uint32_t r = 0; r < nRanges; r++) {
        if (rangeEnd[r] > Q->n || rangeBegin[r] > rangeEnd[r]) return s->fail(SD_EINVAL, "sd_search_stream: bad range");
        uint32_t c0 = rangeBegin[r];
        if (chunks.empty() && c0 < rangeEnd[r]) {
            Chunk c;
            c.range = r;
            c.c0 = c0;
            c.c1 = (uint32_t) std::min<uint64_t>(rangeEnd[r], (uint64_t) c0 + std::max<uint32_t>(1, std::min(chunkQ, std::max<uint32_t>(1000, chunkQ / 4))));
            chunks.push_back(c);
            c0 = c.c1;
        }
        const uint32_t left = rangeEnd[r] - c0;
        const uint32_t parts = (left + chunkQ - 1) / chunkQ;
        for (uint32_t x = 0; x < parts; x++) {
            Chunk c;
            c.range = r;
            c.c0 = c0;
            c.c1 = c0 + left / parts + (x < left % parts ? 1u : 0u);
            chunks.push_back(c);
            c0 = c.c1;
        }
    }
    std::vector<int64_t> lastChunkOf(nRanges, -1);
    for (size_t x = 0; x < chunks.size(); x++) lastChunkOf[chunks[x].range] = (int64_t) x;

    StageThread biasStage{"sd-bias"}, pfStage{"sd-pf0"}, aggStage{"sd-agg"};
    double *tm = s->seconds;

    auto biasJob = [s, Q, profile](uint32_t c0, uint32_t c1) {
        std::unique_ptr<BiasOut> o(new BiasOut());
        const double cpu0 = threadCpuSec();
        o->c0 = c0;
        o->c1 = c1;
        const uint32_t nq = c1 - c0;
        const uint64_t r0 = Q->offsets[c0], r1 = Q->offsets[c1];
        o->off.resize((size_t) nq + 1);
        for (uint32_t i = 0; i <= nq; i++) o->off[i] = Q->offsets[c0 + i] - r0;
        if (profile) {
            o->cpu = threadCpuSec() - cpu0;
            return o;
        }
        const double t0 = nowSec();
        o->sw.assign(r1 - r0 + 1, 0);
        if (s->ungapped) {
            if (s->par.compBiasCorr) o->rc = sd_host_sw_comp_bias(s->host, 0, Q->residues + r0, o->off.data(), nq, o->sw.data());
            o->seconds = nowSec() - t0;
            o->cpu = threadCpuSec() - cpu0;
            return o;
        }
        o->dg.assign(r1 - r0 + 1, 0);
        o->km.assign(r1 - r0 + 1, 0);
        if (s->par.compBiasCorr) {
            if (s->ctxBias)
// ... 518 lines not shown
```

Measured before the change: 2955.

## Pair reverse-pass SW tasks sharing a query onto one profile via start-row offsets

Adds a 'shared start' form of the packed int16 aligned score kernel for the reverse (start-finding) pass. Tasks from the same query with different end rows now share a single full query profile in one wavefront. Each task gets a per-lane starting segment whose profile entries are masked to a neutral value, and the boundary input is cut with a hand-off mask. Pairing keys are extended so only the new start classes get grouped. This halves profile builds and keeps both wavefront halves busy, at the cost of computing masked rows that contribute nothing. It is enabled by default through an environment-controlled context flag.

```diff
diff --git a/include/spacedust_gpu.h b/include/spacedust_gpu.h
--- a/include/spacedust_gpu.h
+++ b/include/spacedust_gpu.h
@@ -96,6 +96,7 @@
 int sd_sw_download_bytes(sd_ctx *ctx, uint64_t *recordBytes, uint64_t *poolBytes);
 
 int sd_sw_set_narrow_final(sd_ctx *ctx, int on);
+int sd_sw_set_shared_start(sd_ctx *ctx, int on);
 
 int sd_selftest_sort_pairs(sd_ctx *ctx, const uint32_t *keys, const uint32_t *vals, uint32_t n, int beginBit, int endBit, uint32_t *outKeys,
                            uint32_t *outVals);
diff --git a/spacedust_amd/_lib.py b/spacedust_amd/_lib.py
--- a/spacedust_amd/_lib.py
+++ b/spacedust_amd/_lib.py
@@ -243,6 +243,7 @@
         'sd_sw_set_cigar_pool': (C.c_int, [_vp, C.c_int]),
         'sd_sw_download_bytes': (C.c_int, [_vp, C.POINTER(C.c_uint64), C.POINTER(C.c_uint64)]),
         'sd_sw_set_narrow_final': (C.c_int, [_vp, C.c_int]),
+        'sd_sw_set_shared_start': (C.c_int, [_vp, C.c_int]),
         'sd_r2p_create': (C.c_int, [C.POINTER(_vp)]),
         'sd_r2p_destroy': (None, [_vp]),
         'sd_r2p_batch': (C.c_int, [_vp, C.POINTER(R2pParams), C.c_uint32] + [_vp] * 12),
diff --git a/spacedust_amd/api.py b/spacedust_amd/api.py
--- a/spacedust_amd/api.py
+++ b/spacedust_amd/api.py
@@ -450,6 +450,9 @@
     def set_narrow_final(self, on=True):
         _check(self.h, self.L.sd_sw_set_narrow_final(self.h, 1 if on else 0), 'sd_sw_set_narrow_final')
 
+    def set_shared_start(self, on=True):
+        _check(self.h, self.L.sd_sw_set_shared_start(self.h, 1 if on else 0), 'sd_sw_set_shared_start')
+
     def sw_download_bytes(self):
         a, b = C.c_uint64(), C.c_uint64()
         self.L.sd_sw_download_bytes(self.h, C.byref(a), C.byref(b))
diff --git a/spacedust_amd/csrc/cli/sd_mod_iter.cpp b/spacedust_amd/csrc/cli/sd_mod_iter.cpp
--- a/spacedust_amd/csrc/cli/sd_mod_iter.cpp
+++ b/spacedust_amd/csrc/cli/sd_mod_iter.cpp
@@ -80,6 +80,7 @@
     ~Worker() {
         if (r2p) sd_r2p_destroy(r2p);
         if (ctx) sd_sw_set_narrow_final(ctx, 0);
+        if (ctx) sd_sw_set_shared_start(ctx, 0);
         if (ctx) sd_ctx_destroy(ctx);
         if (host) sd_host_destroy(host);
     }
@@ -364,6 +365,7 @@
         if (sd_r2p_create(&W.r2p) != SD_OK) return fail("sd_r2p_create failed");
         if (S.profile) sd_profile_enable(W.ctx, 1);
         sd_sw_set_narrow_final(W.ctx, (getenv("SD_SW_NARROW_FINAL") && atoi(getenv("SD_SW_NARROW_FINAL")) == 0) ? 0 : 1);
+        sd_sw_set_shared_start(W.ctx, (getenv("SD_SW_SHARED_START") && atoi(getenv("SD_SW_SHARED_START")) == 0) ? 0 : 1);
     }
     uint64_t indexEntries = 0;
     TargetH seqTarget, profTarget;
diff --git a/spacedust_amd/csrc/hip/sd_common.h b/spacedust_amd/csrc/hip/sd_common.h
--- a/spacedust_amd/csrc/hip/sd_common.h
+++ b/spacedust_amd/csrc/hip/sd_common.h
@@ -37,6 +37,7 @@
     const sd_sw_result *alignDevRes = nullptr;
     size_t alignDevResN = 0;
     bool cigarPool = false;
+    bool sharedStart = false;
     bool narrowFinal = false;
     uint64_t d2hRecordBytes = 0, d2hPoolBytes = 0;
     hipDeviceProp_t prop;
diff --git a/spacedust_amd/csrc/hip/sd_sw.hip b/spacedust_amd/csrc/hip/sd_sw.hip
--- a/spacedust_amd/csrc/hip/sd_sw.hip
+++ b/spacedust_amd/csrc/hip/sd_sw.hip
@@ -711,13 +711,13 @@
                        t->dRes, dMat, go, ge, dOut, dBound, dOrder, (const int8_t *) q->dProf);
 }
 
-template <int RT, bool SHARED>
+template <int RT, bool SHARED, bool START = false>
 void launchScorePkAligned(sd_ctx *ctx, const SwTask *dTasks, const uint32_t *dOrder, uint32_t n, const sd_seqset *q, const sd_seqset *t,
                           const int8_t *dMat, int go, int ge, int32_t *dOut, uint2 * ) {
     if (n == 0) return;
     constexpr uint32_t perWave = 4;
     dim3 grid((n + perWave - 1) / perWave), block(64);
-    hipLaunchKernelGGL((sdpk::sw_score_pk_aligned_kernel<RT, SHARED>), grid, block, 0, ctx->stream, dTasks, n, q->dRes, q->dBias, t->dRes,
+    hipLaunchKernelGGL((sdpk::sw_score_pk_aligned_kernel<RT, SHARED, START>), grid, block, 0, ctx->stream, dTasks, n, q->dRes, q->dBias, t->dRes,
                        dMat, go, ge, dOut, dOrder, (const int8_t *) q->dProf);
 }
 
@@ -730,7 +730,8 @@
                        go, ge, dOut, dBound, dOrder, (const int8_t *) q->dProf);
 }
 
-enum ScoreKernel { SCORE_PK = 0, SCORE_PK_WIDE = 1, SCORE_INT32 = 2 };
+enum ScoreKernel { SCORE_PK = 0, SCORE_PK_WIDE = 1, SCORE_INT32 = 2, SCORE_PK_START = 3 };
+constexpr int START_ROWS_MIN = 129, START_ROWS_MAX = 768;
 constexpr int SCORE_ROWS_ANY = 0x7FFFFFFF;
 constexpr int I32_STRIP_ROWS = 1024;
 struct ScoreSide { const char *scope; ScoreLaunch launch; };
@@ -783,6 +784,26 @@
     {SCORE_INT32, 256, 0, {"sw_score.rt8", launchScoreIdx<8>}, {"sw_score.rt8", launchScoreIdx<8>}},
     {SCORE_INT32, 512, 0, {"sw_score.rt16", launchScoreIdx<16>}, {"sw_score.rt16", launchScoreIdx<16>}},
     {SCORE_INT32, SCORE_ROWS_ANY, 1, {"sw_score.rt32", launchScoreIdx<32>}, {"sw_score.rt32", launchScoreIdx<32>}},
+    {SCORE_PK_START, 160, 0, {"sw_score_pk.s_seg5", launchScorePkAligned<5, true, true>}, {"sw_score_pk.s_seg5", launchScorePkAligned<5, true, true>}},
+    {SCORE_PK_START, 192, 0, {"sw_score_pk.s_seg6", launchScorePkAligned<6, true, true>}, {"sw_score_pk.s_seg6", launchScorePkAligned<6, true, true>}},
+    {SCORE_PK_START, 224, 0, {"sw_score_pk.s_seg7", launchScorePkAligned<7, true, true>}, {"sw_score_pk.s_seg7", launchScorePkAligned<7, true, true>}},
+    {SCORE_PK_START, 256, 0, {"sw_score_pk.s_seg8", launchScorePkAligned<8, true, true>}, {"sw_score_pk.s_seg8", launchScorePkAligned<8, true, true>}},
+    {SCORE_PK_START, 288, 0, {"sw_score_pk.s_seg9", launchScorePkAligned<9, true, true>}, {"sw_score_pk.s_seg9", launchScorePkAligned<9, true, true>}},
+    {SCORE_PK_START, 320, 0, {"sw_score_pk.s_seg10", launchScorePkAligned<10, true, true>}, {"sw_score_pk.s_seg10", launchScorePkAligned<10, true, true>}},
+    {SCORE_PK_START, 352, 0, {"sw_score_pk.s_seg11", launchScorePkAligned<11, true, true>}, {"sw_score_pk.s_seg11", launchScorePkAligned<11, true, true>}},
+    {SCORE_PK_START, 384, 0, {"sw_score_pk.s_seg12", launchScorePkAligned<12, true, true>}, {"sw_score_pk.s_seg12", launchScorePkAligned<12, true, true>}},
+    {SCORE_PK_START, 416, 0, {"sw_score_pk.s_seg13", launchScorePkAligned<13, true, true>}, {"sw_score_pk.s_seg13", launchScorePkAligned<13, true, true>}},
+    {SCORE_PK_START, 448, 0, {"sw_score_pk.s_seg14", launchScorePkAligned<14, true, true>}, {"sw_score_pk.s_seg14", launchScorePkAligned<14, true, true>}},
+    {SCORE_PK_START, 480, 0, {"sw_score_pk.s_seg15", launchScorePkAligned<15, true, true>}, {"sw_score_pk.s_seg15", launchScorePkAligned<15, true, true>}},
+    {SCORE_PK_START, 512, 0, {"sw_score_pk.s_seg16", launchScorePkAligned<16, true, true>}, {"sw_score_pk.s_seg16", launchScorePkAligned<16, true, true>}},
+    {SCORE_PK_START, 544, 0, {"sw_score_pk.s_seg17", launchScorePkAligned<17, true, true>}, {"sw_score_pk.s_seg17", launchScorePkAligned<17, true, true>}},
+    {SCORE_PK_START, 576, 0, {"sw_score_pk.s_seg18", launchScorePkAligned<18, true, true>}, {"sw_score_pk.s_seg18", launchScorePkAligned<18, true, true>}},
+    {SCORE_PK_START, 608, 0, {"sw_score_pk.s_seg19", launchScorePkAligned<19, true, true>}, {"sw_score_pk.s_seg19", launchScorePkAligned<19, true, true>}},
+    {SCORE_PK_START, 640, 0, {"sw_score_pk.s_seg20", launchScorePkAligned<20, true, true>}, {"sw_score_pk.s_seg20", launchScorePkAligned<20, true, true>}},
+    {SCORE_PK_START, 672, 0, {"sw_score_pk.s_seg21", launchScorePkAligned<21, true, true>}, {"sw_score_pk.s_seg21", launchScorePkAligned<21, true, true>}},
+    {SCORE_PK_START, 704, 0, {"sw_score_pk.s_seg22", launchScorePkAligned<22, true, true>}, {"sw_score_pk.s_seg22", launchScorePkAligned<22, true, true>}},
+    {SCORE_PK_START, 736, 0, {"sw_score_pk.s_seg23", launchScorePkAligned<23, true, true>}, {"sw_score_pk.s_seg23", launchScorePkAligned<23, true, true>}},
+    {SCORE_PK_START, 768, 0, {"sw_score_pk.s_seg24", launchScorePkAligned<24, true, true>}, {"sw_score_pk.s_seg24", launchScorePkAligned<24, true, true>}},
 };
 constexpr uint32_t N_SCORE_CLASSES = sizeof(SCORE_CLASSES) / sizeof(SCORE_CLASSES[0]);
 static_assert(N_SCORE_CLASSES < 63, "class boundaries are found by one 64-lane wavefront; six class bits in the pair key");
@@ -792,6 +813,7 @@
     return ci;
 }
 constexpr uint32_t FIRST_WIDE_CLASS = firstScoreClass(SCORE_PK_WIDE), FIRST_INT32_CLASS = firstScoreClass(SCORE_INT32);
+constexpr uint32_t FIRST_START_CLASS = firstScoreClass(SCORE_PK_START);
 constexpr uint32_t KEY_INVALID = N_SCORE_CLASSES * 1024u;
 constexpr uint64_t scoreBoundMask(int need) {
     uint64_t m = 0;
@@ -799,6 +821,10 @@
     return m;
 }
 constexpr __host__ __device__ uint32_t scoreClassOf(int n, int tL, int kernel, int wideRowLimit) {
+    if (kernel == SCORE_PK_START) {
+        if (n >= START_ROWS_MIN && n <= START_ROWS_MAX && tL <= 65535) return FIRST_START_CLASS + (n + 31) / 32 - 5;
+        kernel = SCORE_PK;
+    }
     if (kernel == SCORE_PK_WIDE && (n < tL ? n : tL) > wideRowLimit) kernel = SCORE_INT32;
     if (kernel == SCORE_INT32 || tL > 65535) return FIRST_INT32_CLASS + (n <= 128 ? 0 : (n <= 256 ? 1 : (n <= 512 ? 2 : 3)));
     const int strips = (n + 511) / 512 < 4 ? (n + 511) / 512 : 4;
@@ -819,10 +845,20 @@
             if (ci >= N_SCORE_CLASSES || SCORE_CLASSES[ci].form != form || n > SCORE_CLASSES[ci].rows) return false;
             if (ci > 0 && SCORE_CLASSES[ci - 1].form == form && n <= SCORE_CLASSES[ci - 1].rows) return false;
         }
+    for (int n = 1; n <= 2049; n++) {
+        const uint32_t ci = scoreClassOf(n, 1, SCORE_PK_START, SCORE_ROWS_ANY);
+        if (n < START_ROWS_MIN || n > START_ROWS_MAX) {
+            if (ci != scoreClassOf(n, 1, SCORE_PK, SCORE_ROWS_ANY)) return false;
+            continue;
+        }
+        if (ci >= N_SCORE_CLASSES || SCORE_CLASSES[ci].form != SCORE_PK_START || n > SCORE_CLASSES[ci].rows) return false;
+        if (SCORE_CLASSES[ci - 1].form == SCORE_PK_START && n <= SCORE_CLASSES[ci - 1].rows) return false;
+    }
     return true;
 }
 static_assert(scoreClassesAreTheTables(), "scoreClassOf: n lies in (rows of the class before, rows of its class] for every n, in every form");
-static_assert(SCORE_CLASSES[N_SCORE_CLASSES - 1].form == SCORE_INT32 && SCORE_CLASSES[FIRST_INT32_CLASS - 1].form == SCORE_PK_WIDE, "forms in order");
+static_assert(SCORE_CLASSES[N_SCORE_CLASSES - 1].form == SCORE_PK_START && SCORE_CLASSES[FIRST_START_CLASS - 1].form == SCORE_INT32 &&
+              SCORE_CLASSES[FIRST_INT32_CLASS - 1].form == SCORE_PK_WIDE, "forms in order");
 __device__ __forceinline__ uint32_t scoreKey(int n, int tL, int kernel, int wideRowLimit = 800) {
     return scoreClassOf(n, tL, kernel, wideRowLimit) * 1024u + (uint32_t) (1023 - min(tL >> 4, 1023));
 }
@@ -833,7 +869,7 @@
     if (tasks.empty()) return SD_OK;
     HostScope hsAll(ctx, "score.total");
     const size_t n = tasks.size();
-    constexpr int N_I32 = N_SCORE_CLASSES - FIRST_INT32_CLASS, NB = N_I32 * 1024;
+    constexpr int N_I32 = FIRST_START_CLASS - FIRST_INT32_CLASS, NB = N_I32 * 1024;
     auto keyOf = [](const SwTask &t) {
         const uint32_t ci = scoreClassOf(t.n, t.tL, SCORE_INT32, 0) - FIRST_INT32_CLASS;
         return ci * 1024u + (uint32_t) (1023 - std::min(t.tL >> 4, 1023));
@@ -1064,7 +1100,8 @@
            const int32_t *__restrict__ out16, const uint8_t *__restrict__ word, const uint32_t *__restrict__ fwdKeys,
            SwTask *__restrict__ tasks, uint32_t *__restrict__ keys, uint32_t *__restrict__ vals,
            sd_sw_result *__restrict__ res, int usePk,
-           const uint8_t *__restrict__ wide ) {
+           const uint8_t *__restrict__ wide ,
+           int sharedStart ) {
     const uint32_t i = blockIdx.x * blockDim.x + threadIdx.x;
     if (i >= nPairs) return;
     vals[i] = i;
@@ -1095,8 +1132,11 @@
     const int lanes = word[i] ? 16 : 32;
     tk.segLen = max(1, (tk.n + lanes - 1) / lanes);
     tk.slot = i; tk.boundOff = 0;
+    const bool start = sharedStart && usePk && !rerun && scoreClassOf(qL, tk.tL, SCORE_PK_START, 0) >= FIRST_START_CLASS;
+    if (start) tk.segLen = qL - 1 - r.qEnd;
     tasks[i] = tk;
-    keys[i] = scoreKey(tk.n, tk.tL, !usePk ? SCORE_INT32 : (rerun ? SCORE_PK_WIDE : SCORE_PK), gp.wideRowLimit);
+    keys[i] = start ? scoreKey(qL, tk.tL, SCORE_PK_START)
+                    : scoreKey(tk.n, tk.tL, !usePk ? SCORE_INT32 : (rerun ? SCORE_PK_WIDE : SCORE_PK), gp.wideRowLimit);
 }
 
 struct TbClass { int cap; const char *scope; };
@@ -1450,12 +1490,17 @@
 
 constexpr uint32_t PAIR_NONE = 0xFFFFFFFFu;
 constexpr int PAIR_QUERY_BITS = 17;
+__host__ __device__ __forceinline__ bool pairedClass(uint32_t ci, int startOnly) {
+    return startOnly ? ci >= FIRST_START_CLASS && ci < N_SCORE_CLASSES : ci < FIRST_INT32_CLASS;
+}
 __global__ void __launch_bounds__(256)
-k_pair_keys(uint32_t n, const uint32_t *__restrict__ keys, const uint32_t *__restrict__ pairQ, uint32_t *__restrict__ key2) {
+k_pair_keys(uint32_t n, const uint32_t *__restrict__ keys, const uint32_t *__restrict__ pairQ, uint32_t *__restrict__ key2, int startOnly) {
     const uint32_t i = blockIdx.x * blockDim.x + threadIdx.x;
     if (i >= n) return;
     const uint32_t k = keys[i];
-    key2[i] = k == KEY_INVALID ? 0xFFFFFFFFu : ((k >> 10) << 26) | (pairQ[i] << 9) | ((k & 1023u) >> 1);
+    uint32_t v = k == KEY_INVALID ? 0xFFFFFFFFu : ((k >> 10) << 26) | (pairQ[i] << 9) | ((k & 1023u) >> 1);
+    if (startOnly && k != KEY_INVALID && !pairedClass(k >> 10, startOnly)) v = ((k >> 10) << 26) | ((k & 1023u) << 16);
+    key2[i] = v;
 }
 __global__ void __launch_bounds__(256)
 k_pair_heads(uint32_t n, const uint32_t *__restrict__ keyS, uint32_t *__restrict__ headPos) {
@@ -1465,11 +1510,12 @@
     headPos[p] = head ? p : 0u;
 }
 __global__ void __launch_bounds__(256)
-k_pair_leaders(uint32_t n, const uint32_t *__restrict__ keyS, const uint32_t *__restrict__ runStart, uint8_t *__restrict__ leader) {
+k_pair_leaders(uint32_t n, const uint32_t *__restrict__ keyS, const uint32_t *__restrict__ runStart, uint8_t *__restrict__ leader,
+               int startOnly) {
     const uint32_t p = blockIdx.x * blockDim.x + threadIdx.x;
     if (p > n) return;
     uint8_t v = 0;
-    if (p < n && (keyS[p] >> 26) < FIRST_INT32_CLASS) {
+    if (p < n && pairedClass(keyS[p] >> 26, startOnly)) {
         const uint32_t o = p - runStart[p];
         v = (o & 1u) == 0 ? 1 : 0;
         const bool lastOfRun = p + 1 >= n || (keyS[p + 1] >> 9) != (keyS[p] >> 9);
@@ -1480,9 +1526,9 @@
 }
 __global__ void __launch_bounds__(256)
 k_pair_emit(uint32_t n, const uint32_t *__restrict__ keyS, const uint32_t *__restrict__ vals, const uint32_t *__restrict__ runStartOf,
-            const uint64_t *__restrict__ pairIdx, uint32_t *__restrict__ order2) {
+            const uint64_t *__restrict__ pairIdx, uint32_t *__restrict__ order2, int startOnly) {
     const uint32_t p = blockIdx.x * blockDim.x + threadIdx.x;
-    if (p >= n || (keyS[p] >> 26) >= FIRST_INT32_CLASS || ((p - runStartOf[p]) & 1u)) return;
+    if (p >= n || !pairedClass(keyS[p] >> 26, startOnly) || ((p - runStartOf[p]) & 1u)) return;
     const uint64_t w = pairIdx[p];
     order2[2 * w] = vals[p];
     const bool mate = p + 1 < n && (keyS[p + 1] >> 9) == (keyS[p] >> 9);
@@ -1519,7 +1565,8 @@
 };
 
 int devRunScore(sd_ctx *ctx, const AlignWs &w, uint32_t nPairs, const uint32_t *dKeys, const sd_seqset *q, const sd_seqset *t, int go, int ge,
-                int32_t *dOut, const uint32_t *dPairQ ) {
+                int32_t *dOut, const uint32_t *dPairQ ,
+                int startOnly = 0 ) {
     const uint32_t *dOrder = w.dOrder;
     const unsigned grid = (nPairs + 255) / 256;
     int rc = SD_OK;
@@ -1538,19 +1585,19 @@
         SD_HIP(ctx, wsGet(ctx, "sp.order2", order2Cap, &dOrder2));
         SD_HIP(ctx, hipMemsetAsync(dOrder2, 0xFF, order2Cap * sizeof(uint32_t), ctx->stream));
         SD_HIP(ctx, wsGet(ctx, "sp.bounds", 64, &dPairBounds));
-        hipLaunchKernelGGL(k_pair_keys, dim3(grid), dim3(256), 0, ctx->stream, nPairs, dKeys, dPairQ, dKey2);
+        hipLaunchKernelGGL(k_pair_keys, dim3(grid), dim3(256), 0, ctx->stream, nPairs, dKeys, dPairQ, dKey2, startOnly);
         rc = devSortPairs(ctx, dKey2, w.dKeysS, w.dVals, dVals2, nPairs, 32);
         if (rc != SD_OK) return rc;
         dOrder = dVals2;
         hipLaunchKernelGGL(k_pair_heads, dim3(grid), dim3(256), 0, ctx->stream, nPairs, w.dKeysS, dHead);
         rc = devInclusiveMax(ctx, dHead, dRunStart, nPairs);
         if (rc != SD_OK) return rc;
-        hipLaunchKernelGGL(k_pair_leaders, dim3((nPairs + 256) / 256), dim3(256), 0, ctx->stream, nPairs, w.dKeysS, dRunStart, dLeader);
+        hipLaunchKernelGGL(k_pair_leaders, dim3((nPairs + 256) / 256), dim3(256), 0, ctx->stream, nPairs, w.dKeysS, dRunStart, dLeader, startOnly);
         rc = devExclusiveScan(ctx, (const uint8_t *) dLeader, dPairIdx, (size_t) nPairs + 1);
         if (rc != SD_OK) return rc;
-        hipLaunchKernelGGL(k_pair_emit, dim3(grid), dim3(256), 0, ctx->stream, nPairs, w.dKeysS, dVals2, dRunStart, dPairIdx, dOrder2);
+        hipLaunchKernelGGL(k_pair_emit, dim3(grid), dim3(256), 0, ctx->stream, nPairs, w.dKeysS, dVals2, dRunStart, dPairIdx, dOrder2, startOnly);
         hipLaunchKernelGGL(k_pair_bounds, dim3(1), dim3(64), 0, ctx->stream, w.dKeysS, nPairs, dPairIdx, dPairBounds,
-                           (int) FIRST_INT32_CLASS + 1);
+                           (int) N_SCORE_CLASSES + 1);
         hipLaunchKernelGGL(k_bounds, dim3(1), dim3(64), 0, ctx->stream, w.dKeysS, nPairs, 1u << 26, w.dBounds, (int) N_SCORE_CLASSES + 1);
     } else {
         rc = devSortPairs(ctx, dKeys, w.dKeysS, w.dVals, w.dOrder, nPairs, 16);
@@ -1562,7 +1609,7 @@
     rc = devExclusiveScan(ctx, w.dScanA, w.dScanB, (size_t) nPairs + 1);
     if (rc != SD_OK) return rc;
     hipLaunchKernelGGL(k_bound_apply, dim3(grid), dim3(256), 0, ctx->stream, nPairs, w.dTasks, w.dScanB);
-    uint32_t hb[N_SCORE_CLASSES + 1], hpb[FIRST_INT32_CLASS + 1];
+    uint32_t hb[N_SCORE_CLASSES + 1], hpb[N_SCORE_CLASSES + 1];
     uint64_t boundTotal = 0;
     if (dPairQ) SD_HIP(ctx, sdD2H(ctx, hpb, dPairBounds, sizeof(hpb)));
     SD_HIP(ctx, sdD2H(ctx, hb, w.dBounds, sizeof(hb)));
@@ -1573,7 +1620,7 @@
     for (uint32_t ci = 0; ci < N_SCORE_CLASSES; ci++) {
         const uint32_t begin = hb[ci], cnt = hb[ci + 1] - hb[ci];
         if (cnt == 0) continue;
-        const bool shared = dPairQ != nullptr && ci < FIRST_INT32_CLASS;
+        const bool shared = dPairQ != nullptr && pairedClass(ci, startOnly);
         const ScoreSide &side = shared ? SCORE_CLASSES[ci].shared : SCORE_CLASSES[ci].unshared;
         ProfScope ps(ctx, side.scope);
         if (shared)
@@ -2402,10 +2449,11 @@
     rc = devRunScore(ctx, w, nPairs, w.dKeys, queries, targets, go, ge, w.dOut16, dShare);
     if (rc != SD_OK) return rc;
     hs.reset(new HostScope(ctx, "align.rev"));
+    const bool sharedStart = ctx->sharedStart && usePk && dShare != nullptr;
     hipLaunchKernelGGL(k_gate_rev, dim3(grid), dim3(256), 0, ctx->stream, nPairs, gp, w.dPQ, w.dPT, queries->dOff, targets->dOff, w.dOut32,
-                       w.dOut16, w.dWord, w.dFwdKeys, w.dTasks, w.dRevKeys, w.dVals, w.dRes, usePk, (const uint8_t *) dWide);
+                       w.dOut16, w.dWord, w.dFwdKeys, w.dTasks, w.dRevKeys, w.dVals, w.dRes, usePk, (const uint8_t *) dWide, sharedStart ? 1 : 0);
     hipLaunchKernelGGL(k_cells, dim3(grid), dim3(256), 0, ctx->stream, nPairs, w.dTasks, w.dRevKeys, w.dCells + 1);
-    rc = devRunScore(ctx, w, nPairs, w.dRevKeys, queries, targets, go, ge, w.dOutRev, nullptr);
+    rc = devRunScore(ctx, w, nPairs, w.dRevKeys, queries, targets, go, ge, w.dOutRev, sharedStart ? dShare : nullptr, 1);
     if (rc != SD_OK) return rc;
     hs.reset(new HostScope(ctx, "align.traceback"));
     hipLaunchKernelGGL(k_gate_tb, dim3(grid), dim3(256), 0, ctx->stream, nPairs, gp, w.dPQ, w.dPT, queries->dOff, targets->dOff, w.dOutRev,
@@ -2444,6 +2492,12 @@
 int sd_sw_set_narrow_final(sd_ctx *ctx, int on) {
     if (!ctx) return SD_EINVAL;
     ctx->narrowFinal = on != 0;
+    return SD_OK;
+}
+
+int sd_sw_set_shared_start(sd_ctx *ctx, int on) {
+    if (!ctx) return SD_EINVAL;
+    ctx->sharedStart = on != 0;
     return SD_OK;
 }
 
@@ -2521,9 +2575,9 @@
 }
 
 int sd_selftest_score_class(int kernel, int32_t n, int32_t tL, int shared, int32_t wideRowLimit, uint32_t *klass, char *scope, size_t cap) {
-    if (kernel < SCORE_PK || kernel > SCORE_INT32 || n < 1 || tL < 1 || !klass || (cap && !scope)) return SD_EINVAL;
+    if (kernel < SCORE_PK || kernel > SCORE_PK_START || n < 1 || tL < 1 || !klass || (cap && !scope)) return SD_EINVAL;
     const uint32_t ci = scoreClassOf(n, tL, kernel, wideRowLimit);
-    const ScoreSide &side = shared && ci < FIRST_INT32_CLASS ? SCORE_CLASSES[ci].shared : SCORE_CLASSES[ci].unshared;
+    const ScoreSide &side = shared && (ci < FIRST_INT32_CLASS || ci >= FIRST_START_CLASS) ? SCORE_CLASSES[ci].shared : SCORE_CLASSES[ci].unshared;
     *klass = ci;
     if (cap) snprintf(scope, cap, "%s", side.scope);
     return SD_OK;
diff --git a/spacedust_amd/csrc/hip/sd_sw_pk.h b/spacedust_amd/csrc/hip/sd_sw_pk.h
--- a/spacedust_amd/csrc/hip/sd_sw_pk.h
+++ b/spacedust_amd/csrc/hip/sd_sw_pk.h
@@ -361,7 +361,7 @@
     return r;
 }
 
-template <int RT, bool SHARED>
+template <int RT, bool SHARED, bool START = false>
 __global__ void __launch_bounds__(64)
 sw_score_pk_aligned_kernel(const SwTask *__restrict__ tasks, uint32_t nTasks, const uint8_t *__restrict__ qRes,
                            const int8_t *__restrict__ qBias, const uint8_t *__restrict__ tRes, const int8_t *__restrict__ mat,
@@ -375,6 +375,7 @@
     constexpr int NT = 2 * NGRP;
     constexpr uint32_t ROWB = PSTRIDE * 4;
     static_assert(22 * ROWB < 65536, "row offsets travel in 16 bits");
+    static_assert(SHARED || !START, "the start-row form has one profile per wavefront");
     __shared__ uint32_t prof[SHARED ? 1 : NT][22][PSTRIDE];
     __shared__ int8_t smat[441];
     for (int i = threadIdx.x; i < 441; i += 64) smat[i] = mat[i];
@@ -389,7 +390,7 @@
         if (tid != 0xFFFFFFFFu) {
             tk[x] = tasks[tid];
         } else {
-            tk[x].n = 0; tk[x].tL = 0; tk[x].qOff = 0; tk[x].tOff = 0; tk[x].qStep = 1; tk[x].tStep = 1; tk[x].segLen = 1;
+            tk[x].n = 0; tk[x].tL = 0; tk[x].qOff = 0; tk[x].tOff = 0; tk[x].qStep = 1; tk[x].tStep = 1; tk[x].segLen = START ? 0 : 1;
             tk[x].slot = 0; tk[x].boundOff = 0;
         }
     }
@@ -417,6 +418,8 @@
 #pragma unroll
     for (int x = 0; x < (SHARED ? 1 : 2); x++) {
         const SwTask &T = SHARED ? tk[0] : (x ? B : A);
+        const int64_t pOff = START ? (int64_t) T.qOff - (int64_t) T.segLen * T.qStep : (int64_t) T.qOff;
+        const int pN = START ? T.n + T.segLen : T.n;
         uint32_t *pw = &prof[SHARED ? 0 : 2 * grp + x][0][0] + l * WORDS;
 #pragma unroll
         for (int w = 0; w < WORDS; w++) {
@@ -426,12 +429,12 @@
 #pragma unroll
             for (int b = 0; b < 4; b++) {
                 const int qi = q0 + 4 * w + b;
-                valid[b] = (4 * w + b < RT) && qi < T.n;
+                valid[b] = (4 * w + b < RT) && qi < pN;
                 res[b] = 20;
                 cb[b] = 0;
                 pidx[b] = 0;
                 if (valid[b]) {
-                    const int64_t idx = (int64_t) T.qOff + (int64_t) qi * T.qStep;
+                    const int64_t idx = pOff + (int64_t) qi * T.qStep;
                     res[b] = qRes[idx];
                     cb[b] = qBias[idx];
                     pidx[b] = idx * 21;
@@ -476,6 +479,18 @@
     }
     uint32_t outG = 0, outFf = 0, prevInG = 0;
     uint32_t bestcm = 0, bestcol = 0;
+    const int sA = START ? A.segLen / RT : 0, sB = START ? B.segLen / RT : 0;
+    uint32_t handMask = 0xFFFFFFFFu, keepA[WORDS], keepB[WORDS];
+    const uint32_t neutralWord = 0xC0C0C0C0u;
+    if (START) {
+        handMask = (l == sA ? 0u : 0x0000FFFFu) | (l == sB ? 0u : 0xFFFF0000u);
+#pragma unroll
+        for (int w = 0; w < WORDS; w++) {
+            const int dropA = min(max(A.segLen - sA * RT - 4 * w, 0), 4), dropB = min(max(B.segLen - sB * RT - 4 * w, 0), 4);
+            keepA[w] = l != sA ? 0xFFFFFFFFu : (dropA == 4 ? 0u : 0xFFFFFFFFu << (8 * dropA));
+            keepB[w] = l != sB ? 0xFFFFFFFFu : (dropB == 4 ? 0u : 0xFFFFFFFFu << (8 * dropB));
+        }
+    }
     constexpr uint32_t NEUT = (uint32_t) PK_NEUTRAL * ROWB;
     auto loadChunk = [&](int c0) -> uint32_t {
         const int col = c0 + l;
@@ -517,13 +532,20 @@
             }
         }
         uint32_t inG = dppShr1(outG), inFf = dppShr1(outFf);
-        inG = writeLane<32>(0, inG);
-        inFf = writeLane<32>(0, inFf);
+        if (START) {
+            inG &= handMask;
+            inFf &= handMask;
+        } else {
+            inG = writeLane<32>(0, inG);
+            inFf = writeLane<32>(0, inFf);
+        }
         uint32_t h[RTP];
 #pragma unroll
         for (int w = 0; w < WORDS; w++) {
             const uint32_t d0 = (w == 0) ? prevInG : H[4 * w - 1];
-            addProfile4(pac[w], pbc[w], d0, H[4 * w], H[4 * w + 1], H[4 * w + 2], h[4 * w], h[4 * w + 1], h[4 * w + 2], h[4 * w + 3]);
+            const uint32_t qa = START ? bfiAsm(keepA[w], pac[w], neutralWord) : pac[w];
+            const uint32_t qb = START ? bfiAsm(keepB[w], pbc[w], neutralWord) : pbc[w];
+            addProfile4(qa, qb, d0, H[4 * w], H[4 * w + 1], H[4 * w + 2], h[4 * w], h[4 * w + 1], h[4 * w + 2], h[4 * w + 3]);
         }
         prevInG = inG;
         uint32_t Ff = inFf, cm = 0;
@@ -555,10 +577,11 @@
     unsigned long long keyA = 0, keyB = 0;
     {
         const uint32_t vA = (bestcm & 0xFFFFu) >> 5, vB = bestcm >> 21;
-        const uint32_t rowA = (uint32_t) (q0 + 31 - (int) (bestcm & 31u)), rowB = (uint32_t) (q0 + 31 - (int) ((bestcm >> 16) & 31u));
+        const uint32_t rowA = (uint32_t) (q0 + 31 - (int) (bestcm & 31u) - (START ? A.segLen : 0));
+        const uint32_t rowB = (uint32_t) (q0 + 31 - (int) ((bestcm >> 16) & 31u) - (START ? B.segLen : 0));
         const uint32_t colA = (bestcol & 0xFFFFu) - (uint32_t) l, colB = (bestcol >> 16) - (uint32_t) l;
-        if (vA > 0) keyA = ((unsigned long long) vA << 40) | ((unsigned long long) (0xFFFFFu - colA) << 20) | (unsigned long long) (0xFFFFFu - rowA);
-        if (vB > 0) keyB = ((unsigned long long) vB << 40) | ((unsigned long long) (0xFFFFFu - colB) << 20) | (unsigned long long) (0xFFFFFu - rowB);
+        if (vA > 0 && l >= sA) keyA = ((unsigned long long) vA << 40) | ((unsigned long long) (0xFFFFFu - colA) << 20) | (unsigned long long) (0xFFFFFu - rowA);
+        if (vB > 0 && l >= sB) keyB = ((unsigned long long) vB << 40) | ((unsigned long long) (0xFFFFFu - colB) << 20) | (unsigned long long) (0xFFFFFu - rowB);
     }
 #pragma unroll
     for (int off = LW / 2; off >= 1; off >>= 1) {
diff --git a/spacedust_amd/csrc/host/sd_search.cpp b/spacedust_amd/csrc/host/sd_search.cpp
--- a/spacedust_amd/csrc/host/sd_search.cpp
+++ b/spacedust_amd/csrc/host/sd_search.cpp
@@ -486,6 +486,17 @@
                 if (c) sd_sw_set_narrow_final(c, 0);
         }
     } narrowFinalMode(s, !(getenv("SD_SW_NARROW_FINAL") && atoi(getenv("SD_SW_NARROW_FINAL")) == 0));
+    struct SharedStartMode {
+        sd_ctx *al[4];
+        explicit SharedStartMode(sd_search *s_, bool on) : al{s_->ctxAl, s_->ctxAl2, s_->ctxAlMore[0], s_->ctxAlMore[1]} {
+            for (sd_ctx *c : al)
+                if (c) sd_sw_set_shared_start(c, on ? 1 : 0);
+        }
+        ~SharedStartMode() {
+            for (sd_ctx *c : al)
+                if (c) sd_sw_set_shared_start(c, 0);
+        }
+    } sharedStartMode(s, !(getenv("SD_SW_SHARED_START") && atoi(getenv("SD_SW_SHARED_START")) == 0));
     std::vector<uint32_t> qSetSize(Q->nSets, 0);
     if (aggregate)
         for (uint32_t i = 0; i < Q->n; i++)
```

Result: faster. 3044, median of 6 (+3.0%).
